# vstroebel/jpeg-encoder

Measured on NVIDIA B200. Metric: megapixels/sec encoded, byte-identical to the reference restatement, higher is better.
Workload: dtype u8 in / i32 arithmetic / i16 coefficients

## Files before the change

jpeg_encoder_b200/csrc/api.cu:

```cuda
#include <cuda.h>
#include <cuda_runtime.h>

#include <climits>
#include <cstdint>
#include <cstdio>
#include <cstdlib>
#include <algorithm>
#include <cstring>
#include <string>
#include <condition_variable>
#include <mutex>
#include <thread>
#include <utility>
#include <vector>

#include "../../include/jpegenc_b200.h"
#include "copy_pool.h"
#include "host.h"
#include "kernels.h"

using namespace jpgb;

namespace {

bool poison_alloc() {
    const char *e = std::getenv("JPGB_POISON_ALLOC");
    return e && e[0] == '1';
}

template <bool kPinned>
struct Buf {
    void *p = nullptr;
    size_t cap = 0;
    Buf() = default;
    Buf(Buf &&o) noexcept : p(std::exchange(o.p, nullptr)), cap(std::exchange(o.cap, 0)) {}
    Buf &operator=(Buf o) noexcept {
        std::swap(p, o.p);
        std::swap(cap, o.cap);
        return *this;
    }
    ~Buf() { if (p) kPinned ? cudaFreeHost(p) : cudaFree(p); }
    cudaError_t reserve(size_t bytes) {
        if (bytes <= cap) return cudaSuccess;
        *this = Buf();
        size_t want = bytes + bytes / 8 + 256;
        if (!kPinned) want = (want + 255) & ~(size_t)255;
        cudaError_t e = kPinned ? cudaMallocHost(&p, want) : cudaMalloc(&p, want);
        if (e != cudaSuccess) return p = nullptr, e;
        cap = want;
        if (poison_alloc()) {
            if (kPinned) std::memset(p, 0xFF, want);
            else if ((e = cudaMemset(p, 0xFF, want)) == cudaSuccess) e = cudaDeviceSynchronize();
        }
        return e;
    }
    template <typename T>
    T *as() const { return static_cast<T *>(p); }
};
using DevBuf = Buf<false>;
using PinnedBuf = Buf<true>;

struct PlanSig {
    jpgb_params p;
    jpgb_strip strip;
    uint32_t is_strip, planar;
};
inline PlanSig plan_sig(const Plan &plan) {
    PlanSig s;
    std::memset(&s, 0, sizeof(s));
    s.p.width = plan.p.width;
    s.p.height = plan.p.height;
    s.p.color_type = plan.p.color_type;
    s.p.quality = plan.p.quality;
    s.p.sampling = plan.p.sampling & 0x7F;
    for (int t = 0; t < 2; ++t) {
        s.p.qtable_kind[t] = plan.p.qtable_kind[t];
        if (plan.p.qtable_kind[t] == JPGB_QT_CUSTOM) std::memcpy(s.p.qtable_custom[t], plan.p.qtable_custom[t], sizeof(s.p.qtable_custom[t]));
    }
    s.p.progressive_scans = plan.p.progressive_scans;
    s.p.optimize_huffman = plan.p.optimize_huffman;
    s.p.restart_interval = plan.p.restart_interval;
    if (plan.is_strip) {
        s.strip.strip_index = plan.strip.strip_index;
        s.strip.n_strips = plan.strip.n_strips;
        s.strip.first_row = plan.strip.first_row;
        s.strip.rows = plan.strip.rows;
        s.strip.full_height = plan.strip.full_height;
    }
    s.is_strip = plan.is_strip;
    s.planar = plan.planar;
    return s;
}
struct CapKey {
    PlanSig sig;
    uint64_t raw_bytes;
    uint32_t n, pad;
};

struct Caps { uint64_t ustream, out, pool_units; };

struct GraphKey {
    PlanSig sig;
    uint64_t words[39];
};

struct GraphCache {
    struct Slot {
        cudaGraphExec_t exec = nullptr;
        GraphKey key{};
        uint32_t launches = 0;
        uint64_t used = 0;
    } slots[4];
    uint64_t clock = 0;
    bool ok = true;
    ~GraphCache() {
        for (Slot &s : slots)
            if (s.exec) cudaGraphExecDestroy(s.exec);
    }
    template <typename Enqueue>
    cudaError_t replay(const GraphKey &key, cudaStream_t st, uint32_t &launches, Enqueue &&enqueue, bool &replayed) {
        Slot *slot = nullptr, *victim = &slots[0];
        for (Slot &g : slots) {
            if (g.exec && std::memcmp(&g.key, &key, sizeof(key)) == 0) slot = &g;
            if (!g.exec || (victim->exec && g.used < victim->used)) victim = &g;
        }
        if (!slot) {
            if (victim->exec) cudaGraphExecDestroy(victim->exec), victim->exec = nullptr;
            const uint32_t launches_before = launches;
            cudaGraph_t graph = nullptr;
            const bool capturing = cudaStreamBeginCapture(st, cudaStreamCaptureModeThreadLocal) == cudaSuccess;
            const int rc = capturing ? enqueue() : JPGB_ERR_CUDA;
            if (capturing && cudaStreamEndCapture(st, &graph) == cudaSuccess && rc == JPGB_OK && graph &&
                cudaGraphInstantiate(&victim->exec, graph, 0) == cudaSuccess) {
                victim->key = key;
                victim->launches = launches - launches_before;
                slot = victim;
            } else {
                victim->exec = nullptr;
                ok = false;
            }
            if (graph) cudaGraphDestroy(graph);
            launches = launches_before;
            cudaGetLastError();
        }
        if (!slot) return cudaSuccess;
        slot->used = ++clock;
        const cudaError_t e = cudaGraphLaunch(slot->exec, st);
        if (e == cudaSuccess) launches += slot->launches, replayed = true;
        return e;
    }
};

}

struct jpgb_encoder {
    int device = 0;
    cudaStream_t stream = nullptr;
    bool own_stream = false;
    std::string err;
    DevBuf pixels, coef, huff, hdr, hdr_len, scratch, pool, chunk_bits, chunk_pool, chunk_bitpos, seglen, segpos, ustream, ffcount, ffpos,
        out, scan_tmp, hist, piece_off, out2, pixels2, status, hdr_parts;
    std::vector<uint8_t> last_tables;
    double ucap_ratio = 0;
    double pool_ratio = 0;
    PinnedBuf h_small, h_hist, h_tables, h_pieces, h_out, h_stage[2];
    cudaEvent_t ev_stage[2] = {};
    bool stage_busy[2] = {};
    CopyPool copy_pool;
    cudaStream_t s_h2d = nullptr, s_d2h = nullptr;
    std::vector<cudaEvent_t> ev_slice;
    cudaEvent_t ev_in[2] = {}, ev_out[2] = {}, ev_enc[2] = {};
    cudaEvent_t ev_wait = nullptr;
    bool timing = false;
    cudaEvent_t ev[JPGB_N_STAGES + 1][2] = {};
    bool ev_used[JPGB_N_STAGES] = {};
    float last_ms[JPGB_N_STAGES] = {};
    bool have_timing = false;
    uint32_t launches = 0;
    uint32_t last_piece_scans = 0;
    bool coef_tagged = false;
    PlanSig coef_sig{};
    const void *coef_pixels = nullptr;
    uint64_t coef_stride = 0;
    float coef_ms[2] = {0.f, 0.f};
    GraphCache graphs;
    bool have_caps = false;
    CapKey cap_key{};
    Caps caps{};
};

namespace {

int fail(jpgb_encoder *e, int code, const std::string &msg) {
    if (e) e->err = msg;
    return code;
}
int fail_cuda(jpgb_encoder *e, cudaError_t ce, const char *what) {
    return fail(e, JPGB_ERR_CUDA, std::string(what) + ": " + cudaGetErrorString(ce));
}
#define CK(call, what)                                        \
    do {                                                      \
        cudaError_t ce__ = (call);                            \
        if (ce__ != cudaSuccess) return fail_cuda(enc, ce__, what); \
    } while (0)

struct StageTimer {
    jpgb_encoder *enc;
    int stage;
    StageTimer(jpgb_encoder *e, int s) : enc(e), stage(s) {
        if (enc->timing) {
            if (!enc->ev_used[stage]) cudaEventRecord(enc->ev[stage][0], enc->stream);
        }
    }
    ~StageTimer() {
        if (enc->timing) {
            cudaEventRecord(enc->ev[stage][1], enc->stream);
            enc->ev_used[stage] = true;
        }
    }
};

void timing_begin(jpgb_encoder *enc) {
    for (int i = 0; i < JPGB_N_STAGES; ++i) enc->ev_used[i] = false;
    enc->have_timing = false;
    enc->launches = 0;
}
void timing_end(jpgb_encoder *enc) {
    if (!enc->timing) return;
    cudaStreamSynchronize(enc->stream);
    for (int i = 0; i < JPGB_N_STAGES; ++i) {
        enc->last_ms[i] = 0.f;
        if (enc->ev_used[i]) cudaEventElapsedTime(&enc->last_ms[i], enc->ev[i][0], enc->ev[i][1]);
    }
    enc->have_timing = true;
}

int validate_and_plan(jpgb_encoder *enc, const jpgb_params *p, size_t len_each, Plan &plan) {
    if (!p) return fail(enc, JPGB_ERR_BAD_PARAMS, "null params");
    if (p->color_type > JPGB_YCCK) return fail(enc, JPGB_ERR_BAD_PARAMS, "bad color_type");
    const size_t required = (size_t)p->width * p->height * (size_t)bytes_per_pixel(p->color_type);
    if (len_each < required) {
        char m[128];
        snprintf(m, sizeof(m), "Image data too small for dimensions and color_type: %zu need at least %zu", len_each, required);
        return fail(enc, JPGB_ERR_BAD_IMAGE_DATA, m);
    }
    const int rc = plan.build(*p);
    if (rc != JPGB_OK) return fail(enc, rc, rc == JPGB_ERR_ZERO_DIMENSIONS ? "Image dimensions must be non zero" : "invalid parameters");
    return JPGB_OK;
}

typedef CUresult (*MemGetAddressRangeFn)(CUdeviceptr *, size_t *, CUdeviceptr);
MemGetAddressRangeFn mem_get_address_range_fn() {
    static MemGetAddressRangeFn fn = [] {
        void *f = nullptr;
        cudaDriverEntryPointQueryResult q;
        if (cudaGetDriverEntryPoint("cuMemGetAddressRange", &f, cudaEnableDefault, &q) != cudaSuccess || q != cudaDriverEntryPointSuccess) f = nullptr;
        return reinterpret_cast<MemGetAddressRangeFn>(f);
    }();
    return fn;
}

int check_device_images(jpgb_encoder *enc, const Plan &plan, const jpgb_device_images &im, uint32_t n) {
    const uint64_t w = plan.p.width, h = plan.p.height;
    const bool planes = im.plane_stride != 0;
    const uint64_t row_bytes = planes ? w : w * (uint64_t)plan.bpp;
    char m[192];
    if (im.row_stride < row_bytes) {
        snprintf(m, sizeof(m), "row_stride %llu is shorter than a row (%llu bytes)", (unsigned long long)im.row_stride, (unsigned long long)row_bytes);
        return fail(enc, JPGB_ERR_BAD_PARAMS, m);
    }
    if (planes && im.plane_stride < w) {
        snprintf(m, sizeof(m), "plane_stride %llu is shorter than a row (%llu bytes)", (unsigned long long)im.plane_stride, (unsigned long long)w);
        return fail(enc, JPGB_ERR_BAD_PARAMS, m);
    }
    const uint8_t ct = plan.p.color_type;
    const uint64_t c_max = !planes ? 0 : (ct == JPGB_LUMA ? 0 : (plan.bpp == 3 || ct == JPGB_RGBA || ct == JPGB_BGRA) ? 2 : 3);
    uint64_t last = 0, t = 0;
    bool over = __builtin_mul_overflow((uint64_t)(n - 1), im.image_stride, &last);
    over |= __builtin_mul_overflow(c_max, im.plane_stride, &t) || __builtin_add_overflow(last, t, &last);
    over |= __builtin_mul_overflow(h - 1, im.row_stride, &t) || __builtin_add_overflow(last, t, &last);
    over |= __builtin_add_overflow(last, row_bytes - 1, &last);
    over |= __builtin_add_overflow((uint64_t)(uintptr_t)im.data, last, &t);
    if (over) return fail(enc, JPGB_ERR_BAD_PARAMS, "the described pixels extend beyond 64-bit addresses");
    CK(cudaSetDevice(enc->device), "cudaSetDevice");
    cudaPointerAttributes attr{};
    const bool known = cudaPointerGetAttributes(&attr, im.data) == cudaSuccess;
    cudaGetLastError();
    if (!known || !(attr.type == cudaMemoryTypeManaged || (attr.type == cudaMemoryTypeDevice && attr.device == enc->device)))
        return fail(enc, JPGB_ERR_BAD_PARAMS, "data is not device or managed memory of the context's device");
    MemGetAddressRangeFn range = mem_get_address_range_fn();
    CUdeviceptr base = 0;
    size_t size = 0;
    if (!range || range(&base, &size, (CUdeviceptr)(uintptr_t)im.data) != CUDA_SUCCESS)
        return fail(enc, JPGB_ERR_BAD_PARAMS, "no allocation is found at data");
    const uint64_t end = (uint64_t)(uintptr_t)im.data + last;
    if (end >= (uint64_t)base + size) {
        snprintf(m, sizeof(m), "the described pixels end %llu bytes past the end of the allocation that holds data",
                 (unsigned long long)(end + 1 - ((uint64_t)base + size)));
        return fail(enc, JPGB_ERR_BAD_PARAMS, m);
    }
    return JPGB_OK;
}

struct HeaderLayout {
    size_t hdr_stride = 0;
    uint32_t head_len = 0, tail_len = 0;
    int n_tables = 0;
};

int setup_header(jpgb_encoder *enc, const Plan &plan, uint32_t n, const uint32_t *given_hist, HeaderLayout &hl) {
    cudaStream_t st = enc->stream;
    const bool optimized = plan.p.optimize_huffman != 0;
    const uint32_t n_huff = optimized ? n : 1;
    const size_t tab_bytes = kHuffWordsPerImage * 4;
    CK(enc->huff.reserve((size_t)n_huff * tab_bytes), "alloc huffman tables");
    CK(enc->hdr_len.reserve((size_t)n_huff * 4), "alloc header lengths");
    std::vector<uint8_t> fresh;
    if (!optimized) {
        HuffTable tables[4];
        default_huffman_tables(reinterpret_cast<HuffTable(*)[2]>(tables));
        std::vector<uint8_t> h = plan.prefix;
        plan.frame_header(reinterpret_cast<const HuffTable(*)[2]>(tables), h);
        h.insert(h.end(), plan.scans[0].sos.begin(), plan.scans[0].sos.end());
        hl.hdr_stride = (h.size() + 15) & ~(size_t)15;
        fresh.assign(tab_bytes + hl.hdr_stride + 4, 0);
        CK(enc->h_tables.reserve(fresh.size()), "alloc tables (host)");
        for (int t = 0; t < 4; ++t)
            if (!tables[t].device_words(t & 1, reinterpret_cast<uint32_t *>(fresh.data() + (size_t)t * 1024)))
                return fail(enc, JPGB_ERR_HUFFMAN, "a Huffman code plus its value bits exceeds 31 bits");
        std::memcpy(fresh.data() + tab_bytes, h.data(), h.size());
        const uint32_t len = (uint32_t)h.size();
        std::memcpy(fresh.data() + tab_bytes + hl.hdr_stride, &len, 4);
    } else {
        std::vector<uint8_t> with;
        {
            HuffTable empty[2][2];
            const uint8_t none[16] = {0};
            for (auto &row : empty)
                for (HuffTable &e : row) e.set(none, nullptr, 0);
            with = plan.prefix;
            plan.frame_header(empty, with);
        }
        hl.n_tables = plan.ncomp >= 3 ? 2 : 1;
        size_t dht_at = plan.prefix.size();
        while (dht_at + 3 < with.size() && !(with[dht_at] == 0xFF && with[dht_at + 1] == 0xC4))
            dht_at += 2 + ((size_t)with[dht_at + 2] << 8 | with[dht_at + 3]);
        fresh.assign(with.begin(), with.begin() + dht_at);
        fresh.insert(fresh.end(), with.begin() + dht_at + (size_t)hl.n_tables * 2 * 21, with.end());
        fresh.insert(fresh.end(), plan.scans[0].sos.begin(), plan.scans[0].sos.end());
        hl.head_len = (uint32_t)dht_at;
        hl.tail_len = (uint32_t)(fresh.size() - dht_at);
        hl.hdr_stride = (fresh.size() + (size_t)hl.n_tables * 2 * (21 + 256) + 15) & ~(size_t)15;
        CK(enc->h_tables.reserve(fresh.size() + 16), "alloc header parts (host)");
        CK(enc->hdr_parts.reserve(fresh.size() + 16), "alloc header parts");
        fresh.push_back(0xA5);
        const size_t hist_words = (size_t)n * 2 * 2 * 257;
        CK(enc->hist.reserve(hist_words * 4), "alloc histogram");
        if (given_hist) {
            CK(enc->h_hist.reserve(hist_words * 4), "alloc histogram (host)");
            CK(cudaStreamSynchronize(st), "staging reuse sync");
            std::memcpy(enc->h_hist.p, given_hist, hist_words * 4);
            CK(cudaMemcpyAsync(enc->hist.p, enc->h_hist.p, hist_words * 4, cudaMemcpyHostToDevice, st), "upload histogram");
        }
    }
    CK(enc->hdr.reserve((size_t)n_huff * hl.hdr_stride), "alloc headers");
    if (enc->last_tables != fresh) {
        CK(cudaStreamSynchronize(st), "staging reuse sync");
        enc->last_tables = fresh;
        const uint8_t *hb = enc->h_tables.as<uint8_t>();
        std::memcpy(enc->h_tables.p, fresh.data(), fresh.size());
        if (!optimized) {
            CK(cudaMemcpyAsync(enc->huff.p, hb, tab_bytes, cudaMemcpyHostToDevice, st), "upload huffman tables");
            CK(cudaMemcpyAsync(enc->hdr.p, hb + tab_bytes, hl.hdr_stride, cudaMemcpyHostToDevice, st), "upload headers");
            CK(cudaMemcpyAsync(enc->hdr_len.p, hb + tab_bytes + hl.hdr_stride, 4, cudaMemcpyHostToDevice, st), "upload header lengths");
        } else {
            CK(cudaMemcpyAsync(enc->hdr_parts.p, hb, hl.head_len + hl.tail_len, cudaMemcpyHostToDevice, st), "upload header parts");
        }
    }
    return JPGB_OK;
}


Caps first_caps(const jpgb_encoder *enc, const CapKey &ck, uint64_t n_chunks) {
    const uint64_t raw_bytes = ck.raw_bytes;
    Caps c;
    c.ustream = (enc->ucap_ratio > 0 ? (uint64_t)(raw_bytes * enc->ucap_ratio) : raw_bytes / 3) + (uint64_t)ck.n * 4096 + 65536;
    c.out = c.ustream + c.ustream / 32 + 4096;
    c.pool_units = (enc->pool_ratio > 0 ? (uint64_t)(raw_bytes * enc->pool_ratio) : raw_bytes / 3) / 16 + n_chunks + 4096;
    if (enc->have_caps && std::memcmp(&enc->cap_key, &ck, sizeof(ck)) == 0) c = enc->caps;
    if (const char *tight = std::getenv("JPGB_TIGHT_CAPS")) {
        const std::string t = std::string(",") + tight + ",";
        if (t.find(",pool,") != std::string::npos) c.pool_units = 1;
        if (t.find(",stream,") != std::string::npos) c.ustream = kStuffChunk;
        if (t.find(",out,") != std::string::npos) c.out = 4096;
    }
    return c;
}

void grow_caps(Caps &c, const unsigned long long *status, uint64_t pool_used) {
    const uint64_t ubytes = status[kStatUnstuffed];
    if (status[kStatFlags] & kFlagPool) c.pool_units = pool_used + pool_used / 64 + 4096;
    if (status[kStatFlags] & kFlagStream) {
        c.ustream = ubytes + ubytes / 16 + 65536;
        c.out = c.ustream + c.ustream / 8 + 4096;
    } else if (status[kStatFlags] & kFlagOut) {
        c.out = ubytes + status[kStatDataFF] + 4096;
    }
}

void settle_caps(jpgb_encoder *enc, const CapKey &ck, const Caps &c, uint64_t ubytes, uint64_t total, uint64_t pool_used, uint64_t n_chunks) {
    auto settle = [](uint64_t cap, uint64_t need, uint64_t slack) {
        const uint64_t lo = need + need / 20 + slack / 2, hi = need + need * 2 / 5 + 2 * slack;
        return (cap >= lo && cap <= hi) ? cap : need + need * 3 / 20 + slack;
    };
    enc->cap_key = ck;
    enc->caps.ustream = settle(c.ustream, ubytes, (uint64_t)ck.n * 4096 + 65536);
    enc->caps.out = std::max(settle(c.out, total, 4096), enc->caps.ustream + enc->caps.ustream / 64);
    enc->caps.pool_units = settle(c.pool_units, pool_used, 4096);
    enc->have_caps = true;
    const double raw = (double)std::max<uint64_t>(ck.raw_bytes, 1);
    enc->pool_ratio = std::max(enc->pool_ratio * 0.98, 1.1 * (double)((pool_used > n_chunks ? pool_used - n_chunks : 0) * 16) / raw);
    enc->ucap_ratio = std::max(enc->ucap_ratio * 0.98, 1.15 * (double)ubytes / raw);
}

struct SequenceFlags { bool tables, given_hist, coder, poison, pieces; };

int enqueue_sequence(jpgb_encoder *enc, const Plan &plan, const DevPlan &hp, const EntropyBuffers &b, uint32_t n, const CoderLaunch &coder,
                     const HeaderLayout &hl, const SequenceFlags &f) {
    cudaStream_t st = enc->stream;
    const uint64_t n_chunks = (uint64_t)plan.chunks_per_image * n, n_segs = b.n_segs_total, n_pieces = b.ustream_cap / kStuffChunk;
    const StatusBlock sb = status_block(n, b.ustream_cap);
    unsigned long long *scan_err = b.status + kStatScanError;
    if (f.coder) {
        CK(cudaMemsetAsync(b.status, 0, 2 * kStatusWords * 8 + sb.mask_bytes, st), "clear status and raw mask");
    } else {
        CK(cudaMemsetAsync(b.status, 0, (kStatScanError + 1) * 8, st), "clear status");
        CK(cudaMemsetAsync(b.raw_mask, 0, sb.mask_bytes, st), "clear raw mask");
    }
    if (f.tables) {
        StageTimer t(enc, 1);
        if (!f.given_hist) {
            CK(cudaMemsetAsync(enc->hist.p, 0, (size_t)n * 2 * 2 * 257 * 4, st), "clear histogram");
            CK(launch_histogram(hp, b.coef, n, enc->hist.as<uint32_t>(), st), "histogram launch");
            enc->launches += 1;
        }
        CK(launch_build_tables(enc->hist.as<uint32_t>(), 1, hl.n_tables, n, enc->huff.as<uint32_t>(), enc->hdr_parts.as<uint8_t>(), hl.head_len,
                               enc->hdr_parts.as<uint8_t>() + hl.head_len, hl.tail_len, enc->hdr.as<uint8_t>(), (uint32_t)hl.hdr_stride,
                               enc->hdr_len.as<uint32_t>(), sb.table_status(b.file_off), st),
           "table build launch");
        enc->launches += 1;
    }
    if (f.coder) {
        StageTimer t(enc, 2);
        CK(launch_encode_chunks(b, hp, n, coder, st), "coding launch");
        enc->launches += 1;
        const bool few_chunks = n_chunks <= 4096, few_segs = n_segs <= 4096;
        if (!few_chunks) CK(launch_exclusive_scan(b.chunk_bits, b.chunk_bitpos, n_chunks, b.scan_tmp, st, &enc->launches, scan_err), "chunk position scan");
        if (few_segs) {
            CK(launch_positions(b, hp, n, few_chunks, st), "positions launch");
            enc->launches += 1;
        } else {
            if (few_chunks) CK(launch_exclusive_scan(b.chunk_bits, b.chunk_bitpos, n_chunks, b.scan_tmp, st, &enc->launches, scan_err), "chunk position scan");
            CK(launch_segment_lengths(b, hp, n, st), "segment length launch");
            CK(launch_exclusive_scan(b.seglen, b.segpos, n_segs, b.scan_tmp, st, &enc->launches, scan_err), "segment position scan");
            enc->launches += 1;
        }
    }
    {
        StageTimer t(enc, 3);
        if (f.poison) CK(cudaMemsetAsync(b.ustream, 0xFF, b.ustream_cap + 64, st), "poison stream");
        CK(launch_segment_leads(b, hp, n, st), "segment lead launch");
        CK(launch_place_chunks(b, hp, n, st), "placement launch");
        enc->launches += 2;
    }
    {
        StageTimer t(enc, 4);
        CK(launch_count_ff(b, st), "count ff launch");
        if (ff_scan_needed(b)) CK(launch_exclusive_scan(b.ffcount, b.ffpos, n_pieces, b.scan_tmp, st, &enc->launches, scan_err), "ff scan");
        CK(launch_stuff_scatter(b, hp, n, f.pieces ? enc->piece_off.as<unsigned long long>() : nullptr, st), "scatter launch");
        enc->launches += 2;
        if (f.pieces)
            CK(cudaMemcpyAsync(enc->h_pieces.p, enc->piece_off.p, (plan.scans.size() + 1) * 8, cudaMemcpyDeviceToHost, st), "read piece offsets");
        CK(cudaMemcpyAsync(enc->h_small.p, b.file_off, sb.readback_bytes(), cudaMemcpyDeviceToHost, st), "read file offsets and status");
    }
    return JPGB_OK;
}

GraphKey graph_key(const jpgb_encoder *enc, const PlanSig &sig, const EntropyBuffers &b, uint32_t n, const CoderLaunch &coder,
                   const HeaderLayout &hl, const SequenceFlags &f) {
    static_assert(sizeof(EntropyBuffers) == 26 * 8, "every field of EntropyBuffers takes part in the graph key");
    GraphKey k{{}, {
        (uint64_t)b.coef, (uint64_t)b.huff, (uint64_t)b.huff_per_image, (uint64_t)b.scratch, (uint64_t)b.pool, b.pool_cap,
        (uint64_t)b.chunk_bits, (uint64_t)b.chunk_pool, (uint64_t)b.chunk_bitpos, (uint64_t)b.seglen, (uint64_t)b.segpos,
        (uint64_t)b.hdr_len, (uint64_t)b.hdr, b.hdr_stride, (uint64_t)b.ustream, (uint64_t)b.raw_mask, (uint64_t)b.ffcount,
        (uint64_t)b.ffpos, (uint64_t)b.out, (uint64_t)b.file_off, (uint64_t)b.scan_tmp, b.ustream_cap, b.out_cap, b.n_segs_total,
        (uint64_t)b.status, b.scan_tmp_bytes,
        coder.grid, coder.smem, coder.scratch_bytes, n,
        (uint64_t)f.tables | (uint64_t)f.given_hist << 1 | (uint64_t)f.coder << 2 | (uint64_t)f.poison << 3 | (uint64_t)f.pieces << 4,
        hl.head_len, hl.tail_len, (uint64_t)hl.n_tables,
        (uint64_t)enc->hist.p, (uint64_t)enc->hdr_parts.p, (uint64_t)enc->piece_off.p, (uint64_t)enc->h_small.p, (uint64_t)enc->h_pieces.p}};
    std::memcpy(&k.sig, &sig, sizeof(sig));
    return k;
}

jpgb_device_images contiguous_images(const Plan &plan, const void *d_pixels, uint64_t image_stride) {
    const uint64_t row = (uint64_t)plan.p.width * (plan.planar ? 1 : plan.bpp);
    return {d_pixels, image_stride, row, plan.planar ? row * plan.p.height : 0};
}

void set_pixel_layout(StageAParams &ap, const Plan &plan, const jpgb_device_images &im) {
    ap.pixels = static_cast<const uint8_t *>(im.data);
    ap.image_stride = im.image_stride;
    ap.row_stride = im.row_stride;
    if (plan.planar) {
        ap.plane_stride = im.plane_stride;
    } else if (im.plane_stride && plan.ncomp > 1) {
        const uint8_t ct = plan.p.color_type;
        const bool bgr = ct == JPGB_BGR || ct == JPGB_BGRA;
        ap.channel_planar = 1;
        ap.plane_stride = im.plane_stride;
        for (int k = 0; k < 4; ++k) ap.plane_of[k] = (bgr && k < 3) ? 2 - k : k;
        if (ct == JPGB_BGR || ct == JPGB_RGBA || ct == JPGB_BGRA) {
            ap.color_type = JPGB_RGB;
            ap.bpp = 3;
        }
    }
}

int encode_device(jpgb_encoder *enc, const Plan &plan, const jpgb_device_images &images, uint32_t n, DevBuf &out,
                  std::vector<uint64_t> &offsets, std::vector<uint64_t> *piece_offsets = nullptr, const uint32_t *given_hist = nullptr,
                  bool coef_ready = false) {
    cudaStream_t st = enc->stream;
    DevPlan hp;
    plan.fill_device_plan(hp);

    const uint64_t n_segs = (uint64_t)plan.segs_per_image * n;
    const uint64_t n_chunks = (uint64_t)plan.chunks_per_image * n;

    CK(enc->coef.reserve(plan.blocks_per_image * n * 128), "alloc coefficients");
    if (!coef_ready) {
        enc->coef_tagged = false;
        StageAParams ap;
        plan.fill_stage_a(ap);
        set_pixel_layout(ap, plan, images);
        ap.coef = enc->coef.as<int16_t>();
        StageTimer t(enc, 0);
        CK(launch_stage_a(ap, n, st), "stage A launch");
        enc->launches += 1;
    }

    HeaderLayout hl;
    int rc = setup_header(enc, plan, n, given_hist, hl);
    if (rc != JPGB_OK) return rc;

    CK(enc->chunk_bits.reserve(n_chunks * 4), "alloc chunk sizes");
    CK(enc->chunk_pool.reserve(n_chunks * 4), "alloc chunk places");
    CK(enc->chunk_bitpos.reserve((n_chunks + 1) * 8), "alloc chunk positions");
    CK(enc->seglen.reserve(n_segs * 4), "alloc seglen");
    CK(enc->segpos.reserve((n_segs + 1) * 8), "alloc segpos");
    CoderLaunch coder{};
    CK(coder_launch_config(hp, n, coder), "coder configuration");
    CK(enc->scratch.reserve(coder.scratch_bytes), "alloc coder scratch");
    CK(enc->h_small.reserve(status_block(n, 0).readback_bytes()), "alloc readback");
    if (piece_offsets) {
        CK(enc->piece_off.reserve((plan.scans.size() + 1) * 8), "alloc piece offsets");
        CK(enc->h_pieces.reserve((plan.scans.size() + 1) * 8), "alloc piece offsets (host)");
    }

    EntropyBuffers b{};
    b.coef = enc->coef.as<int16_t>();
    b.huff = enc->huff.as<uint32_t>();
    b.huff_per_image = plan.p.optimize_huffman != 0 ? 1 : 0;
    b.scratch = enc->scratch.as<uint32_t>();
    b.chunk_bits = enc->chunk_bits.as<uint32_t>();
    b.chunk_pool = enc->chunk_pool.as<uint32_t>();
    b.chunk_bitpos = enc->chunk_bitpos.as<unsigned long long>();
    b.seglen = enc->seglen.as<uint32_t>();
    b.segpos = enc->segpos.as<unsigned long long>();
    b.hdr_len = enc->hdr_len.as<uint32_t>();
    b.hdr = enc->hdr.as<uint8_t>();
    b.hdr_stride = (uint32_t)hl.hdr_stride;
    b.n_segs_total = n_segs;

    CapKey ck;
    std::memset(&ck, 0, sizeof(ck));
    ck.sig = plan_sig(plan);
    ck.raw_bytes = (uint64_t)plan.p.width * plan.p.height * plan.bpp * n;
    ck.n = n;
    Caps caps = first_caps(enc, ck, n_chunks);
    const char *poison_env = std::getenv("JPGB_POISON_STREAM");
    uint64_t ubytes = 0, total = 0, pool_used = 0;
    bool coded = false;
    for (int attempt = 0;; ++attempt) {
        caps.ustream = (caps.ustream + kStuffChunk - 1) / kStuffChunk * kStuffChunk;
        const uint64_t n_pieces = caps.ustream / kStuffChunk;
        const StatusBlock sb = status_block(n, caps.ustream);
        CK(enc->ustream.reserve(caps.ustream + 64), "alloc unstuffed stream");
        CK(enc->status.reserve(sb.bytes()), "alloc status and raw mask");
        CK(enc->ffcount.reserve((n_pieces + 1) * 4), "alloc ff counts");
        CK(enc->ffpos.reserve((n_pieces + 2) * 8), "alloc ff positions");
        CK(enc->scan_tmp.reserve(scan_tmp_bytes(std::max<uint64_t>(n_pieces, std::max(n_chunks, n_segs)))), "alloc scan scratch");
        CK(enc->pool.reserve(caps.pool_units * 16), "alloc chunk pool");
        CK(out.reserve(caps.out + 64), "alloc output");
        b.pool = enc->pool.as<uint32_t>();
        b.pool_cap = caps.pool_units;
        b.ustream = enc->ustream.as<uint8_t>();
        b.file_off = sb.file_off(enc->status.p);
        b.status = sb.status(enc->status.p);
        b.raw_mask = sb.raw_mask(enc->status.p);
        b.ffcount = enc->ffcount.as<uint32_t>();
        b.ffpos = enc->ffpos.as<unsigned long long>();
        b.scan_tmp = enc->scan_tmp.p;
        b.out = out.as<uint8_t>();
        b.ustream_cap = caps.ustream;
        b.out_cap = caps.out;
        const SequenceFlags f{plan.p.optimize_huffman != 0 && attempt == 0, given_hist != nullptr, !coded, poison_env && poison_env[0] == '1',
                              piece_offsets != nullptr};
        auto enqueue = [&] { return enqueue_sequence(enc, plan, hp, b, n, coder, hl, f); };
        bool replayed = false;
        if (attempt == 0 && enc->graphs.ok && !enc->timing)
            CK(enc->graphs.replay(graph_key(enc, ck.sig, b, n, coder, hl, f), st, enc->launches, enqueue, replayed), "graph launch");
        if (!replayed) {
            rc = enqueue();
            if (rc != JPGB_OK) return rc;
        }
        CK(cudaStreamSynchronize(st), "final sync");
        const unsigned long long *status = sb.status(enc->h_small.p);
        if (status[kStatScanError]) return fail(enc, JPGB_ERR_CUDA, "internal: prefix-sum look-back timed out");
        if (status[kStatFlags] & kFlagSegment4G) return fail(enc, JPGB_ERR_BAD_PARAMS, "a scan segment exceeds 4 GiB (use a restart interval)");
        if (f.tables && (sb.table_status(enc->h_small.p)[kStatFlags] & kFlagHuffmanLong))
            return fail(enc, JPGB_ERR_HUFFMAN, "an optimized Huffman code does not fit (longer than 32 bits, or code plus value bits beyond 31)");
        ubytes = status[kStatUnstuffed];
        if (f.coder) pool_used = status[kStatPoolCursor];
        if (status[kStatFlags] == 0) {
            total = ubytes + status[kStatDataFF];
            break;
        }
        if (attempt >= 3) return fail(enc, JPGB_ERR_CUDA, "internal: buffer capacity retry did not converge");
        coded = !(status[kStatFlags] & kFlagPool);
        grow_caps(caps, status, pool_used);
    }
    settle_caps(enc, ck, caps, ubytes, total, pool_used, n_chunks);
    if (piece_offsets) {
        piece_offsets->assign(enc->h_pieces.as<uint64_t>(), enc->h_pieces.as<uint64_t>() + plan.scans.size() + 1);
        enc->last_piece_scans = (uint32_t)plan.scans.size();
    }
    offsets.assign(enc->h_small.as<uint64_t>(), enc->h_small.as<uint64_t>() + n + 1);
    if (offsets[n] != total) return fail(enc, JPGB_ERR_CUDA, "internal: file offsets disagree with stream size");
    return JPGB_OK;
}

constexpr size_t kStageBytes = 16u << 20;
cudaError_t upload_host(jpgb_encoder *enc, void *d_dst, const uint8_t *src, size_t bytes, cudaStream_t s) {
    cudaPointerAttributes attr{};
    const bool pinned = cudaPointerGetAttributes(&attr, src) == cudaSuccess && (attr.type == cudaMemoryTypeHost || attr.type == cudaMemoryTypeManaged);
    cudaGetLastError();
    if (pinned || bytes <= 65536) return cudaMemcpyAsync(d_dst, src, bytes, cudaMemcpyHostToDevice, s);
    size_t piece = kStageBytes;
    if (bytes >= kStageBytes && bytes < 2 * kStageBytes) piece = ((bytes / 2 + (1u << 20) - 1) >> 20) << 20;
    unsigned hw = std::thread::hardware_concurrency();
    if (const char *e = std::getenv("JPGB_COPY_THREADS")) hw = (unsigned)std::max(1, std::atoi(e));
    for (size_t off = 0, k = 0; off < bytes; off += piece, ++k) {
        const int b = (int)(k & 1);
        const size_t n = std::min(piece, bytes - off);
        cudaError_t e = enc->h_stage[b].reserve(kStageBytes);
        if (e != cudaSuccess) return e;
        if (enc->stage_busy[b]) {
            e = cudaEventSynchronize(enc->ev_stage[b]);
            if (e != cudaSuccess) return e;
        }
        unsigned threads = (unsigned)std::min<size_t>(4, n >> 22);
        if (hw && threads > hw) threads = hw;
        enc->copy_pool.copy(enc->h_stage[b].p, src + off, n, threads);
        e = cudaMemcpyAsync(static_cast<uint8_t *>(d_dst) + off, enc->h_stage[b].p, n, cudaMemcpyHostToDevice, s);
        if (e != cudaSuccess) return e;
        e = cudaEventRecord(enc->ev_stage[b], s);
        if (e != cudaSuccess) return e;
        enc->stage_busy[b] = true;
    }
    return cudaSuccess;
}

int encode_host_pipelined(jpgb_encoder *enc, const Plan &plan, const uint8_t *const *pixels, uint32_t n,
                          std::vector<uint64_t> &offsets) {
    const size_t img_bytes = (size_t)plan.p.width * plan.p.height * plan.bpp;
    const size_t stride = (img_bytes + 255) & ~(size_t)255;
    uint32_t chunk = (uint32_t)std::max<size_t>(1, (96u << 20) / stride);
    chunk = std::min(chunk, n);
    const uint32_t n_chunks = (n + chunk - 1) / chunk;
    CK(enc->pixels.reserve(stride * chunk), "alloc pixels");
    if (n_chunks > 1) CK(enc->pixels2.reserve(stride * chunk), "alloc pixels");
    CK(enc->h_out.reserve(std::max<size_t>(img_bytes * n / 3, 1 << 20)), "alloc pinned output");
    offsets.assign(1, 0);
    cudaStream_t st = enc->stream;

    if (n == 1 && !plan.planar && img_bytes >= (48u << 20)) {
        const size_t row_bytes = (size_t)plan.p.width * plan.bpp;
        const uint32_t mcu_px = 8 * plan.vmax;
        uint32_t rows_per_slice = (uint32_t)std::max<size_t>(1, (32u << 20) / (row_bytes * mcu_px));
        rows_per_slice = (rows_per_slice + 3) & ~3u;
        const uint32_t n_slices = (plan.mcu_rows + rows_per_slice - 1) / rows_per_slice;
        CK(enc->pixels.reserve(stride), "alloc pixels");
        CK(enc->coef.reserve(plan.blocks_per_image * 128), "alloc coefficients");
        enc->coef_tagged = false;
        while (enc->ev_slice.size() < n_slices) {
            cudaEvent_t e;
            CK(cudaEventCreateWithFlags(&e, cudaEventDisableTiming), "create event");
            enc->ev_slice.push_back(e);
        }
        StageAParams ap;
        plan.fill_stage_a(ap);
        for (uint32_t k = 0; k < n_slices; ++k) {
            const size_t r0 = (size_t)k * rows_per_slice * mcu_px, r1 = std::min<size_t>(plan.p.height, r0 + (size_t)rows_per_slice * mcu_px);
            CK(upload_host(enc, enc->pixels.as<uint8_t>() + r0 * row_bytes, pixels[0] + r0 * row_bytes, (r1 - r0) * row_bytes, enc->s_h2d), "upload slice");
            CK(cudaEventRecord(enc->ev_slice[k], enc->s_h2d), "record slice");
        }
        for (uint32_t k = 0; k < n_slices; ++k) {
            const size_t r0 = (size_t)k * rows_per_slice * mcu_px, r1 = std::min<size_t>(plan.p.height, r0 + (size_t)rows_per_slice * mcu_px);
            StageAParams sp = ap;
            sp.pixels = enc->pixels.as<uint8_t>() + r0 * row_bytes;
            sp.coef = enc->coef.as<int16_t>();
            sp.image_stride = stride;
            sp.height = (int)(r1 - r0);
            sp.mcu_row0 = (int)(k * rows_per_slice);
            sp.mcu_rows = (int)std::min<uint32_t>(rows_per_slice, plan.mcu_rows - k * rows_per_slice);
            CK(cudaStreamWaitEvent(st, enc->ev_slice[k], 0), "wait slice");
            CK(launch_stage_a(sp, 1, st), "stage A launch");
            enc->launches += 1;
        }
        std::vector<uint64_t> off;
        const int rc = encode_device(enc, plan, contiguous_images(plan, enc->pixels.p, stride), 1, enc->out, off, nullptr, nullptr, true);
        if (rc != JPGB_OK) return rc;
        CK(enc->h_out.reserve(std::max<size_t>(off[1], 1 << 20)), "alloc pinned output");
        CK(cudaMemcpyAsync(enc->h_out.p, enc->out.p, off[1], cudaMemcpyDeviceToHost, st), "download file");
        CK(cudaStreamSynchronize(st), "download sync");
        offsets.push_back(off[1]);
        return JPGB_OK;
    }

    auto upload = [&](uint32_t c) -> cudaError_t {
        DevBuf &px = (c & 1) ? enc->pixels2 : enc->pixels;
        const uint32_t lo = c * chunk, hi = std::min(n, lo + chunk);
        if (c >= 2) {
            cudaError_t e = cudaStreamWaitEvent(enc->s_h2d, enc->ev_enc[c & 1], 0);
            if (e != cudaSuccess) return e;
        }
        for (uint32_t i = lo; i < hi; ++i) {
            cudaError_t e = upload_host(enc, px.as<uint8_t>() + stride * (i - lo), pixels[i], img_bytes, enc->s_h2d);
            if (e != cudaSuccess) return e;
        }
        return cudaEventRecord(enc->ev_in[c & 1], enc->s_h2d);
    };

    {
        StageTimer t(enc, 5);
        CK(upload(0), "upload pixels");
    }
    uint64_t total = 0;
    for (uint32_t c = 0; c < n_chunks; ++c) {
        const uint32_t lo = c * chunk, hi = std::min(n, lo + chunk), cn = hi - lo;
        if (c + 1 < n_chunks) CK(upload(c + 1), "upload pixels");
        DevBuf &px = (c & 1) ? enc->pixels2 : enc->pixels;
        DevBuf &ob = (c & 1) ? enc->out2 : enc->out;
        CK(cudaStreamWaitEvent(st, enc->ev_in[c & 1], 0), "wait upload");
        if (c >= 2) CK(cudaStreamWaitEvent(st, enc->ev_out[c & 1], 0), "wait download");
        std::vector<uint64_t> off;
        const int rc = encode_device(enc, plan, contiguous_images(plan, px.p, stride), cn, ob, off);
        if (rc != JPGB_OK) return rc;
        CK(cudaEventRecord(enc->ev_enc[c & 1], st), "record encode");
        const uint64_t bytes = off[cn];
        if (total + bytes > enc->h_out.cap) {
            CK(cudaStreamSynchronize(enc->s_d2h), "download sync");
            PinnedBuf bigger;
            CK(bigger.reserve((total + bytes) * 2), "grow pinned output");
            std::memcpy(bigger.p, enc->h_out.p, total);
            std::swap(enc->h_out, bigger);
        }
        CK(cudaMemcpyAsync(enc->h_out.as<uint8_t>() + total, ob.p, bytes, cudaMemcpyDeviceToHost, enc->s_d2h), "download files");
        CK(cudaEventRecord(enc->ev_out[c & 1], enc->s_d2h), "record download");
        for (uint32_t i = 0; i < cn; ++i) offsets.push_back(total + off[i + 1]);
        total += bytes;
    }
    {
        StageTimer t(enc, 6);
        CK(cudaStreamSynchronize(enc->s_d2h), "download sync");
    }
    return JPGB_OK;
}

int encode_host_batch(jpgb_encoder *enc, const jpgb_params *p, const uint8_t *const *pixels, size_t len_each, uint32_t n,
                      uint8_t **outs, size_t *out_lens, const uint8_t **pinned_base, uint64_t *pinned_offsets) {
    if (!enc) return JPGB_ERR_BAD_PARAMS;
    const bool pinned_api = pinned_base != nullptr;
    if (!pixels || n == 0 || (pinned_api ? !pinned_offsets : (!outs || !out_lens))) return fail(enc, JPGB_ERR_BAD_PARAMS, "null argument");
    if (!pinned_api)
        for (uint32_t i = 0; i < n; ++i) outs[i] = nullptr, out_lens[i] = 0;
    Plan plan;
    int rc = validate_and_plan(enc, p, len_each, plan);
    if (rc != JPGB_OK) return rc;
    CK(cudaSetDevice(enc->device), "cudaSetDevice");
    const bool was_timing = enc->timing;
    enc->timing = false;
    timing_begin(enc);
    std::vector<uint64_t> off;
    rc = encode_host_pipelined(enc, plan, pixels, n, off);
    enc->timing = was_timing;
    if (rc != JPGB_OK) return rc;
    if (pinned_api) {
        *pinned_base = enc->h_out.as<uint8_t>();
        std::memcpy(pinned_offsets, off.data(), (size_t)(n + 1) * 8);
        return JPGB_OK;
    }
    for (uint32_t i = 0; i < n; ++i) {
        const size_t sz = (size_t)(off[i + 1] - off[i]);
        outs[i] = static_cast<uint8_t *>(std::malloc(sz ? sz : 1));
        if (!outs[i]) {
            for (uint32_t k = 0; k < i; ++k) std::free(outs[k]), outs[k] = nullptr;
            return fail(enc, JPGB_ERR_NOMEM, "out of host memory");
        }
        out_lens[i] = sz;
        std::memcpy(outs[i], enc->h_out.as<uint8_t>() + off[i], sz);
    }
    return JPGB_OK;
}

}

extern "C" {

void jpgb_params_default(jpgb_params *p, uint8_t quality) {
    std::memset(p, 0, sizeof(*p));
    p->quality = quality;
    p->sampling = quality < 90 ? 0x22 : 0x11;
    p->density_unit = 0;
    p->density_x = p->density_y = 1;
}

int jpgb_encoder_create(int device, void *cuda_stream, jpgb_encoder **out) {
    if (!out) return JPGB_ERR_BAD_PARAMS;
    *out = nullptr;
    int count = 0;
    if (cudaGetDeviceCount(&count) != cudaSuccess || device < 0 || device >= count) return JPGB_ERR_CUDA;
    cudaDeviceProp prop;
    if (cudaGetDeviceProperties(&prop, device) != cudaSuccess) return JPGB_ERR_CUDA;
    if (prop.major != 10) return JPGB_ERR_CUDA;
    if (cudaSetDevice(device) != cudaSuccess) return JPGB_ERR_CUDA;
    jpgb_encoder *e = new (std::nothrow) jpgb_encoder();
    if (!e) return JPGB_ERR_NOMEM;
    e->device = device;
    if (cuda_stream) {
        e->stream = static_cast<cudaStream_t>(cuda_stream);
    } else {
        if (cudaStreamCreateWithFlags(&e->stream, cudaStreamNonBlocking) != cudaSuccess) {
            delete e;
            return JPGB_ERR_CUDA;
        }
        e->own_stream = true;
    }
    for (int i = 0; i < JPGB_N_STAGES; ++i)
        for (int k = 0; k < 2; ++k) cudaEventCreate(&e->ev[i][k]);
    cudaStreamCreateWithFlags(&e->s_h2d, cudaStreamNonBlocking);
    cudaStreamCreateWithFlags(&e->s_d2h, cudaStreamNonBlocking);
    for (int i = 0; i < 2; ++i) {
        cudaEventCreateWithFlags(&e->ev_in[i], cudaEventDisableTiming);
        cudaEventCreateWithFlags(&e->ev_out[i], cudaEventDisableTiming);
        cudaEventCreateWithFlags(&e->ev_enc[i], cudaEventDisableTiming);
        cudaEventCreateWithFlags(&e->ev_stage[i], cudaEventDisableTiming);
    }
    cudaEventCreateWithFlags(&e->ev_wait, cudaEventDisableTiming);
    *out = e;
    return JPGB_OK;
}

void jpgb_encoder_destroy(jpgb_encoder *e) {
    if (!e) return;
    cudaSetDevice(e->device);
    cudaStreamSynchronize(e->stream);
    if (e->s_h2d) cudaStreamDestroy(e->s_h2d);
    if (e->s_d2h) cudaStreamDestroy(e->s_d2h);
    for (cudaEvent_t ev : e->ev_slice) cudaEventDestroy(ev);
    for (int i = 0; i < 2; ++i) {
        if (e->ev_in[i]) cudaEventDestroy(e->ev_in[i]);
        if (e->ev_out[i]) cudaEventDestroy(e->ev_out[i]);
        if (e->ev_enc[i]) cudaEventDestroy(e->ev_enc[i]);
        if (e->ev_stage[i]) cudaEventDestroy(e->ev_stage[i]);
    }
    if (e->ev_wait) cudaEventDestroy(e->ev_wait);
    for (int i = 0; i < JPGB_N_STAGES; ++i)
        for (int k = 0; k < 2; ++k)
            if (e->ev[i][k]) cudaEventDestroy(e->ev[i][k]);
    if (e->own_stream) cudaStreamDestroy(e->stream);
    delete e;
}

const char *jpgb_last_error(const jpgb_encoder *e) { return e ? e->err.c_str() : "no encoder"; }

int jpgb_encode(jpgb_encoder *enc, const jpgb_params *p, const uint8_t *pixels, size_t len, uint8_t **out, size_t *out_len) {
    if (!out || !out_len) return JPGB_ERR_BAD_PARAMS;
    *out = nullptr;
    *out_len = 0;
    const uint8_t *px[1] = {pixels};
    return encode_host_batch(enc, p, px, len, 1, out, out_len, nullptr, nullptr);
}

void jpgb_free(void *buf) { std::free(buf); }

static int encode_planar_pinned(jpgb_encoder *enc, const jpgb_params *p, const uint8_t *const planes[4], size_t plane_len, size_t *out_len) {
    if (!p || !planes) return fail(enc, JPGB_ERR_BAD_PARAMS, "null argument");
    const uint8_t ct = p->color_type;
    if (ct != JPGB_LUMA && ct != JPGB_YCBCR && ct != JPGB_CMYK && ct != JPGB_YCCK)
        return fail(enc, JPGB_ERR_BAD_PARAMS, "planar input takes a JPEG colour type: Luma, Ycbcr, Cmyk or Ycck");
    const size_t plane_bytes = (size_t)p->width * p->height;
    if (plane_len < plane_bytes) return fail(enc, JPGB_ERR_BAD_IMAGE_DATA, "plane shorter than width*height");
    Plan plan;
    plan.planar = true;
    const int rc = plan.build(*p);
    if (rc != JPGB_OK) return fail(enc, rc, rc == JPGB_ERR_ZERO_DIMENSIONS ? "Image dimensions must be non zero" : "invalid parameters");
    CK(cudaSetDevice(enc->device), "cudaSetDevice");
    timing_begin(enc);
    const size_t stride = (plane_bytes * plan.ncomp + 255) & ~(size_t)255;
    CK(enc->pixels.reserve(stride), "alloc planes");
    for (int c = 0; c < plan.ncomp; ++c) {
        if (!planes[c]) return fail(enc, JPGB_ERR_BAD_PARAMS, "null plane");
        CK(upload_host(enc, enc->pixels.as<uint8_t>() + plane_bytes * c, planes[c], plane_bytes, enc->stream), "upload plane");
    }
    std::vector<uint64_t> off;
    const int rc2 = encode_device(enc, plan, contiguous_images(plan, enc->pixels.p, stride), 1, enc->out, off);
    if (rc2 != JPGB_OK) return rc2;
    const size_t sz = (size_t)off[1];
    CK(enc->h_out.reserve(sz ? sz : 1), "alloc pinned output");
    CK(cudaMemcpyAsync(enc->h_out.p, enc->out.p, sz, cudaMemcpyDeviceToHost, enc->stream), "download file");
    CK(cudaStreamSynchronize(enc->stream), "download sync");
    *out_len = sz;
    timing_end(enc);
    return JPGB_OK;
}

int jpgb_encode_planar(jpgb_encoder *enc, const jpgb_params *p, const uint8_t *const planes[4], size_t plane_len, uint8_t **out,
                       size_t *out_len) {
    if (!enc) return JPGB_ERR_BAD_PARAMS;
    if (!out || !out_len) return fail(enc, JPGB_ERR_BAD_PARAMS, "null argument");
    *out = nullptr;
    *out_len = 0;
    size_t sz = 0;
    const int rc = encode_planar_pinned(enc, p, planes, plane_len, &sz);
    if (rc != JPGB_OK) return rc;
    *out = static_cast<uint8_t *>(std::malloc(sz ? sz : 1));
    if (!*out) return fail(enc, JPGB_ERR_NOMEM, "out of host memory");
    std::memcpy(*out, enc->h_out.p, sz);
    *out_len = sz;
    return JPGB_OK;
}

int jpgb_encode_planar_to_sink(jpgb_encoder *enc, const jpgb_params *p, const uint8_t *const planes[4], size_t plane_len,
                               jpgb_write_all_fn write_all, void *user) {
    if (!enc) return JPGB_ERR_BAD_PARAMS;
    if (!write_all) return fail(enc, JPGB_ERR_BAD_PARAMS, "null sink");
    size_t sz = 0;
    const int rc = encode_planar_pinned(enc, p, planes, plane_len, &sz);
    if (rc != JPGB_OK) return rc;
    if (write_all(user, enc->h_out.as<uint8_t>(), sz) != 0) return fail(enc, JPGB_ERR_SINK, "sink write_all failed");
    return JPGB_OK;
}

int jpgb_encode_to_sink(jpgb_encoder *enc, const jpgb_params *p, const uint8_t *pixels, size_t len, jpgb_write_all_fn write_all,
                        void *user) {
    if (!enc) return JPGB_ERR_BAD_PARAMS;
    if (!write_all) return fail(enc, JPGB_ERR_BAD_PARAMS, "null sink");
    const uint8_t *px[1] = {pixels};
    const uint8_t *files = nullptr;
    uint64_t offs[2] = {0, 0};
    const int rc = encode_host_batch(enc, p, px, len, 1, nullptr, nullptr, &files, offs);
    if (rc != JPGB_OK) return rc;
    if (write_all(user, files + offs[0], (size_t)(offs[1] - offs[0])) != 0) return fail(enc, JPGB_ERR_SINK, "sink write_all failed");
    return JPGB_OK;
}

int jpgb_encode_batch(jpgb_encoder *enc, const jpgb_params *p, const uint8_t *const *pixels, size_t len_each, uint32_t n,
                      uint8_t **outs, size_t *out_lens) {
    return encode_host_batch(enc, p, pixels, len_each, n, outs, out_lens, nullptr, nullptr);
}

int jpgb_encode_batch_pinned(jpgb_encoder *enc, const jpgb_params *p, const uint8_t *const *pixels, size_t len_each, uint32_t n,
                             const uint8_t **files, uint64_t *offsets) {
    if (!files) return JPGB_ERR_BAD_PARAMS;
    return encode_host_batch(enc, p, pixels, len_each, n, nullptr, nullptr, files, offsets);
}

int jpgb_encode_batch_device(jpgb_encoder *enc, const jpgb_params *p, const void *d_pixels, size_t image_stride, uint32_t n,
                             const void **d_files, uint64_t *offsets) {
    if (!enc) return JPGB_ERR_BAD_PARAMS;
    if (!d_pixels || !d_files || !offsets || n == 0) return fail(enc, JPGB_ERR_BAD_PARAMS, "null argument");
    Plan plan;
    int rc = validate_and_plan(enc, p, image_stride, plan);
    if (rc != JPGB_OK) return rc;
    CK(cudaSetDevice(enc->device), "cudaSetDevice");
    timing_begin(enc);
    std::vector<uint64_t> off;
    rc = encode_device(enc, plan, contiguous_images(plan, d_pixels, image_stride), n, enc->out, off);
    if (rc != JPGB_OK) return rc;
    timing_end(enc);
    std::memcpy(offsets, off.data(), (size_t)(n + 1) * 8);
    *d_files = enc->out.p;
    return JPGB_OK;
}

int jpgb_encode_batch_device_strided(jpgb_encoder *enc, const jpgb_params *p, const jpgb_device_images *images, uint32_t n,
                                     const void **d_files, uint64_t *offsets) {
    if (!enc) return JPGB_ERR_BAD_PARAMS;
    enc->launches = 0;
    if (!images || !images->data || !d_files || !offsets || n == 0) return fail(enc, JPGB_ERR_BAD_PARAMS, "null argument");
    Plan plan;
    int rc = validate_and_plan(enc, p, SIZE_MAX, plan);
    if (rc != JPGB_OK) return rc;
    rc = check_device_images(enc, plan, *images, n);
    if (rc != JPGB_OK) return rc;
    plan.planar = images->plane_stride != 0 && (p->color_type == JPGB_YCBCR || p->color_type == JPGB_YCCK);
    timing_begin(enc);
    std::vector<uint64_t> off;
    rc = encode_device(enc, plan, *images, n, enc->out, off);
    if (rc != JPGB_OK) return rc;
    timing_end(enc);
    std::memcpy(offsets, off.data(), (size_t)(n + 1) * 8);
    *d_files = enc->out.p;
    return JPGB_OK;
}

int jpgb_encoder_wait_stream(jpgb_encoder *enc, void *stream) {
    if (!enc) return JPGB_ERR_BAD_PARAMS;
    cudaStream_t s = static_cast<cudaStream_t>(stream);
    if (s == enc->stream) return JPGB_OK;
    CK(cudaSetDevice(enc->device), "cudaSetDevice");
    CK(cudaEventRecord(enc->ev_wait, s), "record the caller's stream");
    CK(cudaStreamWaitEvent(enc->stream, enc->ev_wait, 0), "wait for the caller's stream");
    return JPGB_OK;
}

int jpgb_scan_count(const jpgb_params *p, uint32_t *n_scans) {
    if (!p || !n_scans) return JPGB_ERR_BAD_PARAMS;
    Plan plan;
    const int rc = plan.build(*p);
    if (rc != JPGB_OK) return rc;
    *n_scans = (uint32_t)plan.scans.size();
    return JPGB_OK;
}

int jpgb_plan_strips(const jpgb_params *p, uint32_t max_strips, jpgb_strip *strips, uint32_t *n_strips) {
    if (!p || !strips || !n_strips || max_strips == 0) return JPGB_ERR_BAD_PARAMS;
    Plan plan;
    const int rc = plan.build(*p);
    if (rc != JPGB_OK) return rc;
    const uint32_t R = p->restart_interval;
    if (R == 0) return JPGB_ERR_BAD_PARAMS;
    auto gcd = [](uint64_t a, uint64_t b) { while (b) { const uint64_t t = a % b; a = b; b = t; } return a; };
    uint64_t step = 1;
    for (const Scan &s : plan.scans) {
        const uint64_t upr = s.comp < 0 ? plan.mcu_cols : (uint64_t)plan.comps[s.comp].v * plan.true_w[s.comp];
        const uint64_t need = R / gcd(R, upr);
        step = step / gcd(step, need) * need;
    }
    const uint64_t groups = (plan.mcu_rows + step - 1) / step;
    uint32_t n = (uint32_t)std::min<uint64_t>(max_strips, groups);
    if (n == 0) n = 1;
    const uint32_t rows_per_mcu = 8 * plan.vmax;
    uint64_t g0 = 0;
    for (uint32_t i = 0; i < n; ++i) {
        const uint64_t g1 = groups * (i + 1) / n;
        const uint64_t r0 = g0 * step * rows_per_mcu, r1 = std::min<uint64_t>(g1 * step * rows_per_mcu, p->height);
        strips[i].strip_index = i;
        strips[i].n_strips = n;
        strips[i].first_row = (uint16_t)r0;
        strips[i].rows = (uint16_t)(r1 - r0);
        strips[i].full_height = p->height;
        g0 = g1;
    }
    *n_strips = n;
    return JPGB_OK;
}

static int encode_strip(jpgb_encoder *enc, const jpgb_params *p, const jpgb_strip *strip, const void *d_pixels, const uint32_t *hist_total,
                        const void **d_bytes, uint64_t *piece_offsets) {
    if (!enc) return JPGB_ERR_BAD_PARAMS;
    if (!p || !strip || !d_pixels || !d_bytes || !piece_offsets) return fail(enc, JPGB_ERR_BAD_PARAMS, "null argument");
    if (p->color_type > JPGB_YCCK) return fail(enc, JPGB_ERR_BAD_PARAMS, "bad color_type");
    if ((p->optimize_huffman != 0) != (hist_total != nullptr))
        return fail(enc, JPGB_ERR_BAD_PARAMS, "optimized tables with strips take the whole image's histogram (jpgb_encode_strip_device_optimized); other settings take none");
    Plan plan;
    const int rc = plan.build(*p, strip);
    if (rc != JPGB_OK) return fail(enc, rc, "settings or strip geometry do not allow strip encoding (needs restart intervals aligned in every scan)");
    CK(cudaSetDevice(enc->device), "cudaSetDevice");
    timing_begin(enc);
    std::vector<uint64_t> off, pieces;
    const size_t stride = (size_t)p->width * strip->rows * bytes_per_pixel(p->color_type);
    bool reuse = false;
    if (hist_total && enc->coef_tagged && enc->coef_pixels == d_pixels && enc->coef_stride == uint64_t(stride)) {
        const PlanSig sig = plan_sig(plan);
        reuse = std::memcmp(&sig, &enc->coef_sig, sizeof(sig)) == 0;
    }
    const int rc2 = encode_device(enc, plan, contiguous_images(plan, d_pixels, stride), 1, enc->out, off, &pieces, hist_total, reuse);
    enc->coef_tagged = false;
    if (rc2 != JPGB_OK) return rc2;
    timing_end(enc);
    if (reuse && enc->timing) {
        enc->last_ms[0] += enc->coef_ms[0];
        enc->last_ms[1] += enc->coef_ms[1];
    }
    std::memcpy(piece_offsets, pieces.data(), pieces.size() * 8);
    *d_bytes = enc->out.p;
    return JPGB_OK;
}

int jpgb_encode_strip_device(jpgb_encoder *enc, const jpgb_params *p, const jpgb_strip *strip, const void *d_pixels,
                             const void **d_bytes, uint64_t *piece_offsets) {
    return encode_strip(enc, p, strip, d_pixels, nullptr, d_bytes, piece_offsets);
}

int jpgb_encode_strip_device_optimized(jpgb_encoder *enc, const jpgb_params *p, const jpgb_strip *strip, const void *d_pixels,
                                       const uint32_t hist_total[JPGB_HIST_WORDS], const void **d_bytes, uint64_t *piece_offsets) {
    if (enc && !hist_total) return fail(enc, JPGB_ERR_BAD_PARAMS, "null histogram");
    return encode_strip(enc, p, strip, d_pixels, hist_total, d_bytes, piece_offsets);
}

int jpgb_strip_histogram_device(jpgb_encoder *enc, const jpgb_params *p, const jpgb_strip *strip, const void *d_pixels,
                                uint32_t hist[JPGB_HIST_WORDS], int16_t edge_dc[8]) {
    if (!enc) return JPGB_ERR_BAD_PARAMS;
    if (!p || !strip || !d_pixels || !hist || !edge_dc) return fail(enc, JPGB_ERR_BAD_PARAMS, "null argument");
    if (p->color_type > JPGB_YCCK || !p->optimize_huffman) return fail(enc, JPGB_ERR_BAD_PARAMS, "strip histograms belong to optimized Huffman tables");
    Plan plan;
    const int rc = plan.build(*p, strip);
    if (rc != JPGB_OK) return fail(enc, rc, "settings or strip geometry do not allow strip encoding (needs restart intervals aligned in every scan)");
    CK(cudaSetDevice(enc->device), "cudaSetDevice");
    cudaStream_t st = enc->stream;
    DevPlan hp;
    plan.fill_device_plan(hp);
    StageAParams ap;
    plan.fill_stage_a(ap);
    CK(enc->coef.reserve(plan.blocks_per_image * 128), "alloc coefficients");
    ap.pixels = static_cast<const uint8_t *>(d_pixels);
    ap.coef = enc->coef.as<int16_t>();
    ap.image_stride = (size_t)p->width * strip->rows * bytes_per_pixel(p->color_type);
    timing_begin(enc);
    {
        StageTimer t(enc, 0);
        CK(launch_stage_a(ap, 1, st), "stage A launch");
    }
    const size_t hist_bytes = JPGB_HIST_WORDS * 4;
    CK(enc->hist.reserve(hist_bytes), "alloc histogram");
    CK(enc->h_hist.reserve(hist_bytes + 16), "alloc histogram (host)");
    {
        StageTimer t(enc, 1);
        CK(cudaMemsetAsync(enc->hist.p, 0, hist_bytes, st), "clear histogram");
        CK(launch_histogram(hp, enc->coef.as<int16_t>(), 1, enc->hist.as<uint32_t>(), st), "histogram launch");
    }
    enc->launches = 2;
    CK(cudaMemcpyAsync(enc->h_hist.p, enc->hist.p, hist_bytes, cudaMemcpyDeviceToHost, st), "download histogram");
    int16_t *edge = reinterpret_cast<int16_t *>(enc->h_hist.as<uint8_t>() + hist_bytes);
    std::memset(edge, 0, 16);
    for (int c = 0; c < plan.ncomp; ++c) {
        const uint64_t first = plan.block_off[c], last = plan.block_off[c] + (uint64_t)plan.true_w[c] * plan.true_h[c] - 1;
        CK(cudaMemcpyAsync(edge + c, enc->coef.as<int16_t>() + first * 64, 2, cudaMemcpyDeviceToHost, st), "read edge DC");
        CK(cudaMemcpyAsync(edge + 4 + c, enc->coef.as<int16_t>() + last * 64, 2, cudaMemcpyDeviceToHost, st), "read edge DC");
    }
    CK(cudaStreamSynchronize(st), "histogram sync");
    std::memcpy(hist, enc->h_hist.p, hist_bytes);
    std::memcpy(edge_dc, edge, 16);
    enc->coef_sig = plan_sig(plan);
    enc->coef_pixels = d_pixels;
    enc->coef_stride = uint64_t(ap.image_stride);
    enc->coef_tagged = true;
    timing_end(enc);
    enc->coef_ms[0] = enc->timing ? enc->last_ms[0] : 0.f;
    enc->coef_ms[1] = enc->timing ? enc->last_ms[1] : 0.f;
    return JPGB_OK;
}

int jpgb_merge_strip_histograms(const jpgb_params *p, uint32_t n_strips, const uint32_t hist_sum[JPGB_HIST_WORDS], const int16_t *edge_dc,
                                uint32_t hist_total[JPGB_HIST_WORDS]) {
    if (!p || !hist_sum || !edge_dc || !hist_total || n_strips == 0) return JPGB_ERR_BAD_PARAMS;
    Plan plan;
    const int rc = plan.build(*p);
    if (rc != JPGB_OK) return rc;
    std::memcpy(hist_total, hist_sum, JPGB_HIST_WORDS * 4);
    auto category = [](int diff) {
        int a = (int16_t)diff;
        a = a < 0 ? -a : a;
        int n = 0;
        while (a) ++n, a >>= 1;
        return n;
    };
    for (uint32_t s = 1; s < n_strips; ++s)
        for (int c = 0; c < plan.ncomp; ++c) {
            uint32_t *dc = hist_total + (size_t)plan.comps[c].dc_table * 2 * 257;
            const int first = edge_dc[s * 8 + c], prev_last = edge_dc[(s - 1) * 8 + 4 + c];
            dc[category(first)] -= 1;
            dc[category(first - prev_last)] += 1;
        }
    return JPGB_OK;
}

int jpgb_gather_target_create(jpgb_encoder *enc, size_t capacity, void **d_target, uint8_t ipc_handle[64]) {
    if (!enc) return JPGB_ERR_BAD_PARAMS;
    if (!d_target || !ipc_handle || capacity == 0) return fail(enc, JPGB_ERR_BAD_PARAMS, "null argument");
    static_assert(sizeof(cudaIpcMemHandle_t) == 64, "the C ABI carries the IPC handle as 64 bytes");
    CK(cudaSetDevice(enc->device), "cudaSetDevice");
    void *p = nullptr;
    CK(cudaMalloc(&p, capacity + 64), "alloc gather target");
    cudaIpcMemHandle_t h;
    const cudaError_t ce = cudaIpcGetMemHandle(&h, p);
    if (ce != cudaSuccess) {
        cudaFree(p);
        return fail_cuda(enc, ce, "cudaIpcGetMemHandle");
    }
    std::memcpy(ipc_handle, &h, 64);
    *d_target = p;
    return JPGB_OK;
}

int jpgb_gather_target_open(jpgb_encoder *enc, const uint8_t ipc_handle[64], void **d_target) {
    if (!enc) return JPGB_ERR_BAD_PARAMS;
    if (!d_target || !ipc_handle) return fail(enc, JPGB_ERR_BAD_PARAMS, "null argument");
    CK(cudaSetDevice(enc->device), "cudaSetDevice");
    cudaIpcMemHandle_t h;
    std::memcpy(&h, ipc_handle, 64);
    void *p = nullptr;
    CK(cudaIpcOpenMemHandle(&p, h, cudaIpcMemLazyEnablePeerAccess), "cudaIpcOpenMemHandle (peer access over NVLink)");
    *d_target = p;
    return JPGB_OK;
}

int jpgb_gather_target_close(jpgb_encoder *enc, void *d_target, int opened_from_handle) {
    if (!enc) return JPGB_ERR_BAD_PARAMS;
    if (!d_target) return JPGB_OK;
    CK(cudaSetDevice(enc->device), "cudaSetDevice");
    CK(cudaStreamSynchronize(enc->stream), "sync before releasing the gather target");
    if (opened_from_handle) CK(cudaIpcCloseMemHandle(d_target), "cudaIpcCloseMemHandle");
    else CK(cudaFree(d_target), "free gather target");
    return JPGB_OK;
}

int jpgb_last_piece_offsets_device(jpgb_encoder *enc, const uint64_t **d_offsets, uint32_t *n_scans) {
    if (!enc) return JPGB_ERR_BAD_PARAMS;
    if (!d_offsets || !n_scans || !enc->piece_off.p || enc->last_piece_scans == 0) return fail(enc, JPGB_ERR_BAD_PARAMS, "no strip has been encoded on this context");
    *d_offsets = enc->piece_off.as<uint64_t>();
    *n_scans = enc->last_piece_scans;
    return JPGB_OK;
}

int jpgb_gather_place_pieces(jpgb_encoder *enc, void *d_target, size_t target_capacity, const uint64_t *d_table, uint32_t world, uint32_t rank,
                             uint64_t *d_total) {
    if (!enc) return JPGB_ERR_BAD_PARAMS;
    if (!d_target || !d_table || world == 0 || rank >= world || enc->last_piece_scans == 0) return fail(enc, JPGB_ERR_BAD_PARAMS, "bad gather arguments");
    CK(cudaSetDevice(enc->device), "cudaSetDevice");
    CK(launch_place_pieces(enc->out.as<uint8_t>(), static_cast<uint8_t *>(d_target), target_capacity, reinterpret_cast<const unsigned long long *>(d_table),
                           world, rank, enc->last_piece_scans, reinterpret_cast<unsigned long long *>(d_total), enc->stream),
       "piece placement launch");
    return JPGB_OK;
}

int jpgb_download(jpgb_encoder *enc, const void *d_src, size_t n, void *host_dst) {
    if (!enc) return JPGB_ERR_BAD_PARAMS;
    if (n == 0) return JPGB_OK;
    if (!d_src || !host_dst) return fail(enc, JPGB_ERR_BAD_PARAMS, "null argument");
    CK(cudaSetDevice(enc->device), "cudaSetDevice");
    CK(cudaMemcpyAsync(host_dst, d_src, n, cudaMemcpyDeviceToHost, enc->stream), "download");
    CK(cudaStreamSynchronize(enc->stream), "download sync");
    return JPGB_OK;
}

int jpgb_coef_layout_for(const jpgb_params *p, jpgb_coef_layout *l) {
    if (!p || !l) return JPGB_ERR_BAD_PARAMS;
    Plan plan;
    const int rc = plan.build(*p);
    if (rc != JPGB_OK) return rc;
    std::memset(l, 0, sizeof(*l));
    l->n_components = (uint32_t)plan.ncomp;
    for (int c = 0; c < plan.ncomp; ++c) {
        l->blocks_w[c] = plan.pad_w[c];
        l->blocks_h[c] = plan.pad_h[c];
        l->true_w[c] = plan.true_w[c];
        l->true_h[c] = plan.true_h[c];
        l->block_offset[c] = plan.block_off[c];
        l->slot_base[c] = plan.slot_base[c];
        l->comp_h[c] = plan.comps[c].h;
        l->comp_v[c] = plan.comps[c].v;
    }
    l->blocks_per_image = plan.blocks_per_image;
    l->mcu_order = plan.mode == Mode::Interleaved;
    l->mcu_cols = plan.mcu_cols;
    l->mcu_rows = plan.mcu_rows;
    l->blocks_per_mcu = plan.bpu_interleaved;
    return JPGB_OK;
}

int jpgb_stage_a_device(jpgb_encoder *enc, const jpgb_params *p, const void *d_pixels, size_t image_stride, uint32_t n, void *d_coef) {
    if (!enc) return JPGB_ERR_BAD_PARAMS;
    if (!d_pixels || !d_coef || n == 0) return fail(enc, JPGB_ERR_BAD_PARAMS, "null argument");
    Plan plan;
    const int rc = validate_and_plan(enc, p, image_stride, plan);
    if (rc != JPGB_OK) return rc;
    CK(cudaSetDevice(enc->device), "cudaSetDevice");
    StageAParams ap;
    plan.fill_stage_a(ap);
    ap.pixels = static_cast<const uint8_t *>(d_pixels);
    ap.coef = static_cast<int16_t *>(d_coef);
    ap.image_stride = image_stride;
    enc->launches = 0;
    CK(launch_stage_a(ap, n, enc->stream), "stage A launch");
    enc->launches = 1;
    return JPGB_OK;
}

void jpgb_encoder_set_timing(jpgb_encoder *enc, int enabled) {
    if (enc) enc->timing = enabled != 0;
}
int jpgb_encoder_last_timing(const jpgb_encoder *enc, float ms[JPGB_N_STAGES]) {
    if (!enc || !enc->have_timing) return JPGB_ERR_BAD_PARAMS;
    std::memcpy(ms, enc->last_ms, sizeof(enc->last_ms));
    return JPGB_OK;
}
uint32_t jpgb_encoder_last_launch_count(const jpgb_encoder *enc) { return enc ? enc->launches : 0; }

int jpgb_build_header(const jpgb_params *p, uint8_t *buf, size_t cap, size_t *len) {
    if (!p || !len) return JPGB_ERR_BAD_PARAMS;
    Plan plan;
    const int rc = plan.build(*p);
    if (rc != JPGB_OK) return rc;
    HuffTable huff[2][2];
    default_huffman_tables(huff);
    std::vector<uint8_t> h = plan.prefix;
    plan.frame_header(huff, h);
    h.insert(h.end(), plan.scans[0].sos.begin(), plan.scans[0].sos.end());
    *len = h.size();
    if (buf) std::memcpy(buf, h.data(), std::min(cap, h.size()));
    return JPGB_OK;
}

int jpgb_optimized_huffman_table(const uint32_t freq[257], uint8_t length[16], uint8_t values[256], uint32_t *n_values) {
    if (!freq || !length || !values || !n_values) return JPGB_ERR_BAD_PARAMS;
    HuffTable t;
    if (!t.set_optimized(freq)) return JPGB_ERR_HUFFMAN;
    std::memcpy(length, t.length, 16);
    std::memcpy(values, t.values.data(), t.values.size());
    *n_values = (uint32_t)t.values.size();
    return JPGB_OK;
}

int jpgb_optimized_huffman_tables_device(jpgb_encoder *enc, const uint32_t *freq, uint32_t n, int ac, uint8_t *lengths, uint8_t *values,
                                         uint32_t *n_values, uint32_t *words, int *status) {
    if (!enc) return JPGB_ERR_BAD_PARAMS;
    if (!freq || !lengths || !values || !n_values || !words || !status || n == 0) return fail(enc, JPGB_ERR_BAD_PARAMS, "null argument");
    CK(cudaSetDevice(enc->device), "cudaSetDevice");
    cudaStream_t st = enc->stream;
    DevBuf d_hist, d_words, d_dht, d_len, d_bad;
    std::vector<uint8_t> dht((size_t)n * 277);
    std::vector<uint32_t> len(n), bad(n);
    cudaError_t e = d_hist.reserve((size_t)n * 257 * 4);
    if (e == cudaSuccess) e = d_words.reserve((size_t)n * 1024);
    if (e == cudaSuccess) e = d_dht.reserve((size_t)n * 277);
    if (e == cudaSuccess) e = d_len.reserve((size_t)n * 4);
    if (e == cudaSuccess) e = d_bad.reserve((size_t)n * 4);
    if (e == cudaSuccess) e = cudaMemcpyAsync(d_hist.p, freq, (size_t)n * 257 * 4, cudaMemcpyHostToDevice, st);
    if (e == cudaSuccess) e = launch_build_single_tables(d_hist.as<uint32_t>(), n, ac, d_words.as<uint32_t>(), d_dht.as<uint8_t>(), d_len.as<uint32_t>(), d_bad.as<uint32_t>(), st);
    if (e == cudaSuccess) e = cudaMemcpyAsync(words, d_words.p, (size_t)n * 1024, cudaMemcpyDeviceToHost, st);
    if (e == cudaSuccess) e = cudaMemcpyAsync(dht.data(), d_dht.p, dht.size(), cudaMemcpyDeviceToHost, st);
    if (e == cudaSuccess) e = cudaMemcpyAsync(len.data(), d_len.p, (size_t)n * 4, cudaMemcpyDeviceToHost, st);
    if (e == cudaSuccess) e = cudaMemcpyAsync(bad.data(), d_bad.p, (size_t)n * 4, cudaMemcpyDeviceToHost, st);
    if (e == cudaSuccess) e = cudaStreamSynchronize(st);
    if (e != cudaSuccess) return fail_cuda(enc, e, "device table build");
    for (uint32_t i = 0; i < n; ++i) {
        status[i] = bad[i] ? JPGB_ERR_HUFFMAN : JPGB_OK;
        n_values[i] = bad[i] ? 0 : len[i] - 21;
        std::memcpy(lengths + (size_t)i * 16, dht.data() + (size_t)i * 277 + 5, 16);
        std::memcpy(values + (size_t)i * 256, dht.data() + (size_t)i * 277 + 21, 256);
    }
    return JPGB_OK;
}

const char *jpgb_version(void) { return "jpeg-encoder_b200 0.1 (sm_100a; parity target: jpeg-encoder 0.7.0)"; }

}
```

jpeg_encoder_b200/csrc/entropy.cu:

```cuda

#include "kernels.h"

namespace jpgb {
namespace {

__device__ __forceinline__ int find_scan_by_seg(const DevPlan &P, unsigned s) {
    int lo = 0, hi = P.n_scans - 1;
    while (lo < hi) {
        const int mid = (lo + hi + 1) >> 1;
        if (P.scans[mid].seg_base <= s) lo = mid;
        else hi = mid - 1;
    }
    return lo;
}
__device__ __forceinline__ int find_scan_by_chunk(const DevPlan &P, unsigned c) {
    int lo = 0, hi = P.n_scans - 1;
    while (lo < hi) {
        const int mid = (lo + hi + 1) >> 1;
        if (P.scans[mid].chunk_base <= c) lo = mid;
        else hi = mid - 1;
    }
    return lo;
}

__device__ __forceinline__ void value_code(int v, int &size, uint32_t &bits) {
    const int a = v < 0 ? -v : v;
    int top;
    asm("bfind.u32 %0, %1;" : "=r"(top) : "r"(a));
    size = top + 1;
    uint32_t mask;
    asm("bmsk.clamp.b32 %0, 0, %1;" : "=r"(mask) : "r"(size));
    bits = (uint32_t)(v + (v >> 31)) & mask;
}

__device__ __forceinline__ unsigned nonzero16x2(unsigned x) {
    unsigned r;
    asm("min.u16x2 %0, %1, %2;" : "=r"(r) : "r"(x), "r"(0x00010001u));
    return r;
}

template <int T>
struct BitSink {
    unsigned long long acc = 0;
    int n = 0;
    unsigned off = 0;
    uint32_t *slot0;

    __device__ __forceinline__ BitSink(uint32_t *scratch, int visit) : slot0(scratch + visit) {}
    __device__ __forceinline__ void put(uint32_t code, int len) {
        acc = (acc << len) | code;
        n += len;
        if (n >= 32) {
            n -= 32;
            *reinterpret_cast<uint32_t *>(reinterpret_cast<char *>(slot0) + off) = (uint32_t)(acc >> n);
            off += T * 4;
        }
    }
    __device__ __forceinline__ unsigned finish() {
        if (n > 0) *reinterpret_cast<uint32_t *>(reinterpret_cast<char *>(slot0) + off) = (uint32_t)(acc << (32 - n));
        return off / (T * 4) * 32 + n;
    }
};

constexpr uint32_t kCodeBits = 0x07FFFFFFu;

constexpr int kStageStride = 72;
constexpr int kAsmWordsProg = 3072;

__device__ __forceinline__ unsigned long long zrl_markers(unsigned long long m, int first_ac) {
    const unsigned long long z = m | (1ull << (first_ac - 1));
    unsigned long long s = z;
    s |= s << 1;
    s |= s << 2;
    s |= s << 4;
    const unsigned long long s16 = s | (s << 8);
    const unsigned long long s32 = s16 | (s16 << 16);
    const unsigned long long s48 = s32 | (s16 << 32);
    unsigned long long marks = ((z << 16) & ~s16) | ((z << 32) & ~s32) | ((z << 48) & ~s48);
    const int top = 63 - __clzll((long long)m);
    marks &= top > 0 ? (~0ull >> (64 - top)) : 0ull;
    return marks;
}

template <int BASE, int T>
__device__ __forceinline__ void code_half(unsigned m, int &next, unsigned c_shared, const uint32_t *__restrict__ tab, BitSink<T> &sink) {
#pragma unroll 1
    while (m) {
        int p;
        asm("bfind.u32 %0, %1;" : "=r"(p) : "r"(m));
        unsigned bit;
        asm("bmsk.clamp.b32 %0, %1, 1;" : "=r"(bit) : "r"(p));
        m ^= bit;
        const int k = BASE + 31 - p;
        int v;
        asm("ld.shared.s16 %0, [%1];" : "=r"(v) : "r"(c_shared + 2 * k));
        const int run = k - next;
        next = k + 1;
        int size;
        uint32_t bits;
        value_code(v, size, bits);
        const uint32_t e = (tab + run * 16)[size];
        sink.put((e & kCodeBits) | bits, (int)(e >> 27));
    }
}
template <int T>
__device__ __forceinline__ void code_nonzeros(unsigned lo_rev, unsigned hi_rev, int first_ac, int se, const int16_t *__restrict__ c,
                                              const uint32_t *__restrict__ tab, BitSink<T> &sink) {
    int next = first_ac;
    const unsigned c_shared = (unsigned)__cvta_generic_to_shared(c);
    code_half<0, T>(lo_rev, next, c_shared, tab, sink);
    code_half<32, T>(hi_rev, next, c_shared, tab, sink);
    if (next <= se) {
        const uint32_t e = tab[0];
        sink.put(e & kCodeBits, (int)(e >> 27));
    }
}

struct __align__(16) ItemInfo {
    unsigned long long img, blk0, chunk_index0;
    unsigned v_in_seg0, n_valid, group;
    int done;
};

template <int T, bool FULL>
struct CoderSmem {
    static constexpr int kCoefBytes = T * kStageStride * 2;
    static constexpr int kAsmWords = FULL ? kCoefBytes / 4 : kAsmWordsProg;
    static constexpr int oAsm = FULL ? 0 : kCoefBytes;
    static constexpr int oAc = kCoefBytes + (FULL ? 0 : kAsmWordsProg * 4);
    static constexpr int oDc = oAc + 2048;
    static constexpr int oSlot = oDc + 256;
    static constexpr int oBin = oSlot + 128;
    static constexpr int oNb = oBin + 256;
    static constexpr int oOrder = oNb + T * 4;
    static constexpr int oWsum = oOrder + T * 2;
    static constexpr int oItem = oWsum + 64;
    static constexpr int kBytes = oItem + 2 * 64;
};

__host__ __device__ constexpr int coder_min_ctas(int T, bool full) { return full && T >= 128 ? 1280 / T : 1024 / T; }

template <int T, bool FULL>
__global__ void __launch_bounds__(T, coder_min_ctas(T, FULL)) encode_chunks_kernel(const __grid_constant__ EntropyBuffers b, const __grid_constant__ DevPlan P,
                                                          unsigned long long n_items) {
    using L = CoderSmem<T, FULL>;
    extern __shared__ __align__(16) unsigned char smem[];
    int16_t *coef = reinterpret_cast<int16_t *>(smem);
    uint32_t *asmbuf = reinterpret_cast<uint32_t *>(smem + L::oAsm);
    uint32_t *ac_tab = reinterpret_cast<uint32_t *>(smem + L::oAc);
    uint2 *dc_tab = reinterpret_cast<uint2 *>(smem + L::oDc);
    uint32_t *slot_tab = reinterpret_cast<uint32_t *>(smem + L::oSlot);
    uint32_t *bin = reinterpret_cast<uint32_t *>(smem + L::oBin);
    uint32_t *nbv = reinterpret_cast<uint32_t *>(smem + L::oNb);
    auto visit_meta = [&](int v) { return reinterpret_cast<uint4 *>(smem + v * (kStageStride * 2) + 128); };
    uint16_t *order = reinterpret_cast<uint16_t *>(smem + L::oOrder);
    uint32_t *wsum = reinterpret_cast<uint32_t *>(smem + L::oWsum);
    ItemInfo *items = reinterpret_cast<ItemInfo *>(smem + L::oItem);

    const int tid = threadIdx.x, lane = tid & 31, warp = tid >> 5;
    uint32_t *scratch = b.scratch + (size_t)blockIdx.x * (T * kSlotWords);
    long long tab_img = -1;
    for (int i = tid; i < 64; i += T) bin[i] = 0;
    if (tid < kMaxSlots) slot_tab[tid] = (unsigned)P.comp_tbl[P.slot_comp[tid]] | (unsigned)P.slot_back[tid] << 8 | (unsigned)P.slot_first[tid] << 16;
    auto decode = [&](unsigned long long ticket, ItemInfo &it) {
        it.done = ticket >= n_items;
        if (it.done) return;
        unsigned long long img;
        unsigned r;
        if ((ticket >> 32) == 0) {
            unsigned q;
            divmod((unsigned)ticket, P.div_items, q, r);
            img = q;
        } else {
            img = ticket / P.items_per_image;
            r = (unsigned)(ticket - img * P.items_per_image);
        }
        int g = 0;
        while (g + 1 < P.n_groups && r >= P.groups[g + 1].item_base) ++g;
        const DevGroup &G = P.groups[g];
        unsigned seg, chunk;
        divmod(r - G.item_base, G.div_cps, seg, chunk);
        const unsigned long long seg_start = (unsigned long long)seg * G.seg_visits;
        const unsigned long long v0 = seg_start + (unsigned long long)chunk * T;
        unsigned long long seg_end = seg_start + G.seg_visits;
        if (seg_end > G.n_visits) seg_end = G.n_visits;
        it.img = img;
        it.group = (unsigned)g;
        it.v_in_seg0 = chunk * T;
        it.n_valid = v0 < seg_end ? (unsigned)(seg_end - v0 < (unsigned long long)T ? seg_end - v0 : T) : 0u;
        it.blk0 = img * P.blocks_per_image + G.block_base + v0;
        it.chunk_index0 = img * P.chunks_per_image + (r - G.item_base);
    };
    unsigned long long next_ticket = 0;
    if (tid == 0) {
        decode(atomicAdd(b.status + kStatTicket, 1ull), items[0]);
        next_ticket = atomicAdd(b.status + kStatTicket, 1ull);
    }

    for (unsigned round = 0;; ++round) {
        __syncthreads();
        const ItemInfo it = items[round & 1];
        if (it.done) break;
        if (tid == 0) {
            decode(next_ticket, items[(round & 1) ^ 1]);
            next_ticket = atomicAdd(b.status + kStatTicket, 1ull);
        }
        if (it.n_valid == 0) {
            for (int j = tid; j < P.spg; j += T) {
                const unsigned long long ci = it.chunk_index0 + P.scans[it.group + j * P.n_groups].chunk_base;
                b.chunk_bits[ci] = 0;
                b.chunk_pool[ci] = 0;
            }
            continue;
        }
        const DevGroup &G = P.groups[it.group];
        const bool valid = (unsigned)tid < it.n_valid;

        const long long want_tab = b.huff_per_image ? (long long)it.img : 0;
        if (want_tab != tab_img) {
            const uint32_t *set = b.huff + (size_t)want_tab * kHuffWordsPerImage;
            for (int i = tid; i < 512; i += T) {
                ac_tab[i] = __ldg(set + (i >> 8) * 512 + 256 + (i & 255));
            }
            if (tid < 32) {
                const uint32_t e = __ldg(set + (tid >> 4) * 512 + (tid & 15));
                dc_tab[tid] = make_uint2(e & kCodeBits, e >> 27);
            }
            tab_img = want_tab;
        }

        const int16_t *src_blocks = b.coef + it.blk0 * 64;
        {
            const unsigned pieces = it.n_valid * 8;
            const char *g = reinterpret_cast<const char *>(src_blocks) + (size_t)tid * 16;
            const unsigned d = (unsigned)__cvta_generic_to_shared(coef) + (tid >> 3) * (kStageStride * 2) + (tid & 7) * 16;
            if (it.n_valid == T) {
#pragma unroll
                for (int k = 0; k < 8; ++k)
                    asm volatile("cp.async.cg.shared.global [%0], [%1], 16;" ::"r"(d + k * (T / 8) * (kStageStride * 2)), "l"(g + k * T * 16) : "memory");
            } else {
#pragma unroll
                for (int k = 0; k < 8; ++k)
                    if ((unsigned)(tid + k * T) < pieces)
                        asm volatile("cp.async.cg.shared.global [%0], [%1], 16;" ::"r"(d + k * (T / 8) * (kStageStride * 2)), "l"(g + k * T * 16) : "memory");
            }
            asm volatile("cp.async.wait_all;" ::: "memory");
        }
        __syncthreads();

        unsigned long long m_all = 0;
        int dcdiff = 0, tbl = 0;
        if (valid) {
            const uint4 *mine = reinterpret_cast<const uint4 *>(coef + tid * kStageStride);
            unsigned m_lo = 0, m_hi = 0;
#pragma unroll
            for (int w = 0; w < 8; ++w) {
                const uint4 q = mine[w];
                unsigned byte = __dp2a_lo(nonzero16x2(q.x), 0x0201u, 0u);
                byte = __dp2a_lo(nonzero16x2(q.y), 0x0804u, byte);
                byte = __dp2a_lo(nonzero16x2(q.z), 0x2010u, byte);
                byte = __dp2a_lo(nonzero16x2(q.w), 0x8040u, byte);
                if (w < 4) m_lo |= byte << (8 * w);
                else m_hi |= byte << (8 * (w - 4));
            }
            m_all = (((unsigned long long)m_hi << 32) | m_lo) & ~1ull;
            const unsigned v_in_seg = it.v_in_seg0 + tid;
            unsigned unit = v_in_seg, slot = 0;
            if (G.bpu > 1) divmod(v_in_seg, G.div_bpu, unit, slot);
            const unsigned sinfo = G.comp < 0 ? slot_tab[slot] : ((unsigned)P.comp_tbl[G.comp] | 0x10100u);
            tbl = sinfo & 0xFF;
            const int back = (sinfo >> 8) & 0xFF;
            const bool first_of_comp = (sinfo >> 16) != 0;
            int prev = 0;
            if (!(unit == 0 && first_of_comp)) prev = tid >= back ? (int)coef[(tid - back) * kStageStride] : (int)__ldg(src_blocks + ((long long)tid - back) * 64);
            dcdiff = (int)(int16_t)(coef[tid * kStageStride] - prev);
        }

        for (int j = 0; j < (FULL ? 1 : P.spg); ++j) {
            const DevScan &S = P.scans[it.group + j * P.n_groups];
            const int ss = FULL ? 0 : S.ss, se = FULL ? 63 : S.se;
            const int first_ac = ss == 0 ? 1 : ss;
            unsigned m_lo = 0, m_hi = 0;
            uint32_t first = 0;
            if (valid) {
                if (se > 0) {
                    unsigned long long m = FULL ? m_all : m_all & (~0ull << first_ac) & (~0ull >> (63 - se));
                    m |= zrl_markers(m, first_ac);
                    m_lo = __brev((unsigned)m);
                    m_hi = __brev((unsigned)(m >> 32));
                }
                if (ss == 0) {
                    int size;
                    uint32_t bits;
                    value_code(dcdiff, size, bits);
                    const uint2 e = dc_tab[tbl * 16 + size];
                    first = e.x | bits | e.y << 27;
                }
            }
            *visit_meta(tid) = make_uint4(m_lo, m_hi, first, (unsigned)tbl | (valid ? 0x100u : 0u));
            if (se > 0) {
                const int nnz = __popc(m_lo) + __popc(m_hi);
                const unsigned rank = atomicAdd(&bin[nnz], 1u);
                __syncthreads();
                {
                    const unsigned a = bin[2 * lane], c = bin[2 * lane + 1];
                    unsigned inc = a + c;
#pragma unroll
                    for (int d = 1; d < 32; d <<= 1) {
                        const unsigned o = __shfl_up_sync(0xffffffffu, inc, d);
                        if (lane >= d) inc += o;
                    }
                    const unsigned even = inc - a - c, odd = inc - c;
                    const unsigned e = __shfl_sync(0xffffffffu, even, nnz >> 1), o = __shfl_sync(0xffffffffu, odd, nnz >> 1);
                    order[((nnz & 1) ? o : e) + rank] = (uint16_t)tid;
                }
                __syncthreads();
                for (int i = tid; i < 64; i += T) bin[i] = 0;
            } else {
                order[tid] = (uint16_t)tid;
                __syncthreads();
            }

            if (j == 0) {
                const ItemInfo &nx = items[(round & 1) ^ 1];
                if (!nx.done && (unsigned)tid < nx.n_valid)
                    asm volatile("prefetch.global.L2 [%0];" ::"l"(b.coef + (nx.blk0 + tid) * 64));
            }
            {
                const int src = order[tid];
                const uint4 meta = *visit_meta(src);
                const unsigned inf = meta.w;
                unsigned nb = 0;
                if (inf & 0x100u) {
                    const uint32_t dc_code = meta.z;
                    BitSink<T> sink(scratch, src);
                    sink.put(dc_code & kCodeBits, (int)(dc_code >> 27));
                    if (se > 0) code_nonzeros<T>(meta.x, meta.y, first_ac, se, coef + src * kStageStride, ac_tab + (inf & 0xFF) * 256, sink);
                    nb = sink.finish();
                }
                nbv[src] = nb;
            }
            __syncthreads();

            const unsigned myb = nbv[tid];
            const unsigned nw = (myb + 31) >> 5;
            const uint32_t *mine = scratch + tid;
            uint32_t pre[4];
#pragma unroll
            for (int q = 0; q < 4; ++q) pre[q] = __ldcg(mine + q * T);
            unsigned inc = myb;
#pragma unroll
            for (int d = 1; d < 32; d <<= 1) {
                const unsigned o = __shfl_up_sync(0xffffffffu, inc, d);
                if (lane >= d) inc += o;
            }
            unsigned off = inc - myb, total = 0;
#pragma unroll
            for (int w = 0; w < T / 32; ++w) {
                const unsigned sw = __reduce_add_sync(0xffffffffu, nbv[w * 32 + lane]);
                if (w < warp) off += sw;
                total += sw;
            }
            const unsigned total_words = (total + 31) >> 5;
            const unsigned long long ci = it.chunk_index0 + S.chunk_base;
            const unsigned pool_units = (total_words + 3) >> 2;
            unsigned long long pool_at = 0;
            if (tid == 0) {
                if (pool_units) pool_at = atomicAdd(b.status + kStatPoolCursor, (unsigned long long)pool_units);
                b.chunk_bits[ci] = total;
            }
            for (unsigned wb = 0; wb < total_words; wb += L::kAsmWords) {
                const unsigned nwin = total_words - wb < (unsigned)L::kAsmWords ? total_words - wb : (unsigned)L::kAsmWords;
                for (unsigned i = tid * 4; i < nwin; i += T * 4) *reinterpret_cast<uint4 *>(asmbuf + i) = make_uint4(0, 0, 0, 0);
                __syncthreads();
                if (myb) {
                    const unsigned d0 = off >> 5, dl = (off + myb - 1) >> 5, sft = off & 31;
                    auto word = [&](unsigned q) -> uint32_t {
                        if (q >= nw) return 0u;
                        if (q < 4) return q == 0 ? pre[0] : (q == 1 ? pre[1] : (q == 2 ? pre[2] : pre[3]));
                        return __ldcg(mine + q * T);
                    };
                    if (wb == 0 && dl < nwin) {
                        uint32_t prev = pre[0];
                        atomicOr(asmbuf + d0, prev >> sft);
                        unsigned jw = 1;
                        for (unsigned d = d0 + 1; d < dl; ++d, ++jw) {
                            const uint32_t cur = word(jw);
                            asmbuf[d] = __funnelshift_r(cur, prev, sft);
                            prev = cur;
                        }
                        if (dl > d0) atomicOr(asmbuf + dl, __funnelshift_r(word(jw), prev, sft));
                    } else {
                        const unsigned lo = d0 > wb ? d0 : wb, hi = dl < wb + nwin - 1 ? dl : wb + nwin - 1;
                        if (lo <= hi) {
                            unsigned jw = lo - d0;
                            uint32_t prev = jw > 0 ? word(jw - 1) : 0u;
                            for (unsigned d = lo; d <= hi; ++d, ++jw) {
                                const uint32_t cur = word(jw);
                                atomicOr(asmbuf + (d - wb), __funnelshift_r(cur, prev, sft));
                                prev = cur;
                            }
                        }
                    }
                }
                if (tid == 0 && wb == 0) {
                    if (pool_at + pool_units > b.pool_cap) {
                        atomicOr(b.status + kStatFlags, kFlagPool);
                        pool_at = ~0ull;
                    }
                    wsum[8] = (uint32_t)pool_at;
                    wsum[9] = (uint32_t)(pool_at >> 32);
                    b.chunk_pool[ci] = (uint32_t)pool_at;
                }
                __syncthreads();
                const unsigned long long at = ((unsigned long long)wsum[9] << 32) | wsum[8];
                if (at != ~0ull) {
                    uint4 *dst = reinterpret_cast<uint4 *>(b.pool) + at + (wb >> 2);
                    for (unsigned i = tid; i * 4 < nwin; i += T) dst[i] = reinterpret_cast<const uint4 *>(asmbuf)[i];
                }
                if (wb + L::kAsmWords < total_words || !FULL) __syncthreads();
            }
        }
    }
}

__device__ __forceinline__ unsigned lead_len(const EntropyBuffers &b, const DevPlan &P, unsigned long long img, int k,
                                             unsigned seg_in_scan) {
    if (P.scans[k].rst_base + seg_in_scan > 0) return 2;
    if (k > 0) return P.scans[k].sos_len;
    return b.hdr_len[b.huff_per_image ? img : 0];
}

__global__ void __launch_bounds__(256) segment_len_kernel(const __grid_constant__ EntropyBuffers b, const __grid_constant__ DevPlan P, unsigned long long n_segs) {
    const unsigned long long g = (unsigned long long)blockIdx.x * blockDim.x + threadIdx.x;
    if (g >= n_segs) return;
    const unsigned long long img = g / P.segs_per_image;
    const unsigned s = (unsigned)(g - img * P.segs_per_image);
    const int k = find_scan_by_seg(P, s);
    const DevScan &S = P.scans[k];
    const unsigned i = s - S.seg_base;
    const unsigned cps = P.groups[k % P.n_groups].cps;
    const unsigned long long c0 = img * P.chunks_per_image + S.chunk_base + (unsigned long long)i * cps;
    const unsigned long long bits = b.chunk_bitpos[c0 + cps] - b.chunk_bitpos[c0];
    const unsigned tail = (s == P.segs_per_image - 1 && P.has_eoi) ? 2u : 0u;
    const unsigned long long bytes = lead_len(b, P, img, k, i) + ((bits + 7) >> 3) + tail;
    if (bytes > 0xFFFFFFFFull) atomicOr(b.status + kStatFlags, kFlagSegment4G);
    b.seglen[g] = (unsigned)bytes;
}

__device__ __forceinline__ unsigned long long segment_bytes(const EntropyBuffers &b, const DevPlan &P, unsigned long long g) {
    const unsigned long long img = g / P.segs_per_image;
    const unsigned s = (unsigned)(g - img * P.segs_per_image);
    const int k = find_scan_by_seg(P, s);
    const DevScan &S = P.scans[k];
    const unsigned i = s - S.seg_base;
    const unsigned cps = P.groups[k % P.n_groups].cps;
    const unsigned long long c0 = img * P.chunks_per_image + S.chunk_base + (unsigned long long)i * cps;
    const unsigned long long bits = b.chunk_bitpos[c0 + cps] - b.chunk_bitpos[c0];
    const unsigned tail = (s == P.segs_per_image - 1 && P.has_eoi) ? 2u : 0u;
    return lead_len(b, P, img, k, i) + ((bits + 7) >> 3) + tail;
}

__device__ __forceinline__ unsigned long long cta1024_exclusive(unsigned long long v, unsigned long long *sm, unsigned long long &total) {
    const int lane = threadIdx.x & 31, warp = threadIdx.x >> 5;
    unsigned long long inc = v;
#pragma unroll
    for (int d = 1; d < 32; d <<= 1) {
        const unsigned long long o = __shfl_up_sync(0xffffffffu, inc, d);
        if (lane >= d) inc += o;
    }
    if (lane == 31) sm[warp] = inc;
    __syncthreads();
    if (warp == 0) {
        const unsigned long long w = sm[lane];
        unsigned long long winc = w;
#pragma unroll
        for (int d = 1; d < 32; d <<= 1) {
            const unsigned long long o = __shfl_up_sync(0xffffffffu, winc, d);
            if (lane >= d) winc += o;
        }
        sm[lane] = winc - w;
        if (lane == 31) sm[32] = winc;
    }
    __syncthreads();
    const unsigned long long ex = sm[warp] + inc - v;
    total = sm[32];
    __syncthreads();
    return ex;
}

__global__ void __launch_bounds__(1024) positions_kernel(const __grid_constant__ EntropyBuffers b, const __grid_constant__ DevPlan P, unsigned long long n_chunks,
                                                         unsigned long long n_segs, int scan_chunks) {
    __shared__ unsigned long long sm[33];
    unsigned long long carry = 0, total;
    if (scan_chunks) {
        for (unsigned long long base = 0; base < n_chunks; base += 1024) {
            const unsigned long long i = base + threadIdx.x;
            const unsigned long long ex = cta1024_exclusive(i < n_chunks ? b.chunk_bits[i] : 0ull, sm, total);
            if (i < n_chunks) b.chunk_bitpos[i] = carry + ex;
            carry += total;
        }
        if (threadIdx.x == 0) b.chunk_bitpos[n_chunks] = carry;
        __syncthreads();
    }
    carry = 0;
    for (unsigned long long base = 0; base < n_segs; base += 1024) {
        const unsigned long long g = base + threadIdx.x;
        unsigned long long bytes = 0;
        if (g < n_segs) {
            bytes = segment_bytes(b, P, g);
            if (bytes > 0xFFFFFFFFull) atomicOr(b.status + kStatFlags, kFlagSegment4G);
        }
        const unsigned long long ex = cta1024_exclusive(bytes, sm, total);
        if (g < n_segs) b.segpos[g] = carry + ex;
        carry += total;
    }
    if (threadIdx.x == 0) b.segpos[n_segs] = carry;
}

__device__ __forceinline__ unsigned long long stream_bytes(const EntropyBuffers &b) { return b.segpos[b.n_segs_total]; }
__device__ __forceinline__ bool stream_fits(const EntropyBuffers &b) { return stream_bytes(b) <= b.ustream_cap; }

__device__ __forceinline__ void put_raw(const EntropyBuffers &b, unsigned long long pos, uint8_t byte) {
    b.ustream[pos] = byte;
    atomicOr(b.raw_mask + (pos >> 5), 1u << (pos & 31));
}

__global__ void __launch_bounds__(128) segment_lead_kernel(const __grid_constant__ EntropyBuffers b, const __grid_constant__ DevPlan P, unsigned long long n_segs,
                                                           const unsigned wps) {
    const unsigned long long gw = ((unsigned long long)blockIdx.x * blockDim.x + threadIdx.x) >> 5;
    const unsigned long long g = gw / wps;
    const unsigned slice = (unsigned)(gw - g * wps);
    const int lane = threadIdx.x & 31;
    if (blockIdx.x == 0 && threadIdx.x == 0) {
        const unsigned long long bytes = stream_bytes(b);
        b.status[kStatUnstuffed] = bytes;
        if (bytes > b.ustream_cap) atomicOr(b.status + kStatFlags, kFlagStream);
    }
    if (g >= n_segs || !stream_fits(b)) return;
    const unsigned long long img = g / P.segs_per_image;
    const unsigned s = (unsigned)(g - img * P.segs_per_image);
    const int k = find_scan_by_seg(P, s);
    const DevScan &S = P.scans[k];
    const unsigned i = s - S.seg_base;
    const unsigned long long pos = b.segpos[g];
    {
        const bool eoi = s == P.segs_per_image - 1 && P.has_eoi;
        const unsigned cps = P.groups[k % P.n_groups].cps;
        const unsigned long long c0 = img * P.chunks_per_image + S.chunk_base + (unsigned long long)i * cps;
        const unsigned long long bit0 = b.chunk_bitpos[c0];
        const unsigned long long data0 = pos + lead_len(b, P, img, k, i), data1 = b.segpos[g + 1] - (eoi ? 2u : 0u);
        const unsigned per = (cps + wps) / wps;
        const unsigned q1 = (slice + 1) * per < cps + 1 ? (slice + 1) * per : cps + 1;
        for (unsigned q = slice * per + lane; q < q1; q += 32) {
            const unsigned long long pbit = data0 * 8 + (b.chunk_bitpos[c0 + q] - bit0);
            if ((pbit & 31) == 0) continue;
            const unsigned long long w = pbit >> 5;
            const unsigned long long lo = w * 4 > data0 ? w * 4 : data0, hi = w * 4 + 4 < data1 ? w * 4 + 4 : data1;
            if (lo + 4 == hi) reinterpret_cast<uint32_t *>(b.ustream)[w] = 0u;
            else
                for (unsigned long long x = lo; x < hi; ++x) b.ustream[x] = 0;
        }
    }
    if (slice != 0) return;
    if (S.rst_base + i > 0) {
        if (lane == 0) {
            put_raw(b, pos, 0xFF);
            put_raw(b, pos + 1, (uint8_t)(0xD0 + ((S.rst_base + i - 1) & 7)));
        }
    } else if (k > 0) {
        for (unsigned j = lane; j < S.sos_len; j += 32) put_raw(b, pos + j, P.blob[S.sos_off + j]);
    } else {
        const unsigned long long h = b.huff_per_image ? img : 0;
        const unsigned n = b.hdr_len[h];
        const uint8_t *src = b.hdr + h * b.hdr_stride;
#pragma unroll 4
        for (unsigned j = lane; j < n; j += 32) b.ustream[pos + j] = src[j];
        const unsigned long long w0 = pos >> 5, w1 = (pos + n - 1) >> 5;
        for (unsigned long long w = w0 + lane; w <= w1 && n; w += 32) {
            const unsigned long long lo = w * 32 > pos ? w * 32 : pos, hi = (w + 1) * 32 < pos + n ? (w + 1) * 32 : pos + n;
            const unsigned bits = (unsigned)(hi - lo);
            atomicOr(b.raw_mask + w, (bits == 32 ? 0xFFFFFFFFu : ((1u << bits) - 1u)) << (unsigned)(lo & 31));
        }
    }
    if (s == P.segs_per_image - 1 && P.has_eoi && lane == 0) {
        const unsigned long long end = b.segpos[g + 1];
        put_raw(b, end - 2, 0xFF);
        put_raw(b, end - 1, 0xD9);
    }
}

__global__ void __launch_bounds__(256) place_chunks_kernel(const __grid_constant__ EntropyBuffers b, const __grid_constant__ DevPlan P, unsigned long long n_chunks,
                                                           const unsigned per_warp) {
    if (!stream_fits(b) || (b.status[kStatFlags] & kFlagPool)) return;
    const int lane = threadIdx.x & 31;
    const unsigned long long warps = ((unsigned long long)gridDim.x * blockDim.x) >> 5;
    uint32_t *stream = reinterpret_cast<uint32_t *>(b.ustream);
    for (unsigned long long c0 = (((unsigned long long)blockIdx.x * blockDim.x + threadIdx.x) >> 5) * per_warp; c0 < n_chunks; c0 += warps * per_warp) {
        const unsigned long long c = c0 + lane;
        unsigned my_bits = 0, my_pool = 0;
        unsigned long long my_bitpos = 0;
        if ((unsigned)lane < per_warp && c < n_chunks) {
            const unsigned long long img = c / P.chunks_per_image;
            const unsigned r = (unsigned)(c - img * P.chunks_per_image);
            const int k = find_scan_by_chunk(P, r);
            const DevScan &S = P.scans[k];
            const DevGroup &G = P.groups[k % P.n_groups];
            unsigned seg, q;
            divmod(r - S.chunk_base, G.div_cps, seg, q);
            my_bits = b.chunk_bits[c];
            if (my_bits != 0 || q == 0) {
                const unsigned long long seg_first = b.chunk_bitpos[c - q];
                const unsigned long long data_byte = b.segpos[img * P.segs_per_image + S.seg_base + seg] + lead_len(b, P, img, k, seg);
                my_bitpos = data_byte * 8 + (b.chunk_bitpos[c] - seg_first);
                if (my_bits) my_pool = b.chunk_pool[c];
                if (q == 0) {
                    const unsigned long long seg_bits = b.chunk_bitpos[c + G.cps] - seg_first;
                    const unsigned pad = (unsigned)(-(long long)seg_bits) & 7u;
                    if (pad) {
                        const unsigned long long pbit = data_byte * 8 + seg_bits;
                        const unsigned s2 = (unsigned)(pbit & 31);
                        atomicOr(stream + (pbit >> 5), __byte_perm(((1u << pad) - 1u) << (32 - s2 - pad), 0, 0x0123));
                    }
                }
            }
        }
        unsigned todo = __ballot_sync(0xffffffffu, my_bits != 0);
        while (todo) {
            const int who = __ffs(todo) - 1;
            todo &= todo - 1;
            const unsigned bits = __shfl_sync(0xffffffffu, my_bits, who);
            const unsigned long long bitpos = __shfl_sync(0xffffffffu, my_bitpos, who);
            const uint32_t *src = b.pool + (size_t)__shfl_sync(0xffffffffu, my_pool, who) * 4;
            const unsigned sft = (unsigned)(bitpos & 31);
            uint32_t *dst = stream + (bitpos >> 5);
            const unsigned nw = (bits + 31) >> 5, ndw = (sft + bits + 31) >> 5;
            const bool first_owned = sft == 0, last_owned = ((sft + bits) & 31) == 0;
            uint32_t carry = 0;
            for (unsigned base = 0; base < ndw; base += 128) {
                uint32_t cur[4];
#pragma unroll
                for (int u = 0; u < 4; ++u) {
                    const unsigned d = base + 32 * u + lane;
                    cur[u] = d < nw ? __ldg(src + d) : 0u;
                }
#pragma unroll
                for (int u = 0; u < 4; ++u) {
                    const unsigned d = base + 32 * u + lane;
                    uint32_t prev = __shfl_up_sync(0xffffffffu, cur[u], 1);
                    if (lane == 0) prev = carry;
                    carry = __shfl_sync(0xffffffffu, cur[u], 31);
                    if (d < ndw) {
                        const uint32_t val = sft ? __funnelshift_r(cur[u], prev, sft) : cur[u];
                        const uint32_t be = __byte_perm(val, 0, 0x0123);
                        const bool owned = (d > 0 || first_owned) && (d + 1 < ndw || last_owned);
                        if (owned) dst[d] = be;
                        else atomicOr(dst + d, be);
                    }
                }
            }
        }
    }
}

__device__ __forceinline__ uint32_t ff_flags(uint32_t w) {
    const uint32_t x = ~w;
    const uint32_t t = ((x & 0x7F7F7F7Fu) + 0x7F7F7F7Fu) | x;
    return ~t & 0x80808080u;
}
__device__ __forceinline__ unsigned flags_to_nibble(uint32_t z) { return (((z >> 7) * 0x00204081u) >> 21) & 0xFu; }

__device__ __forceinline__ unsigned ff_bits16(const uint4 d, unsigned raw16, unsigned valid) {
    unsigned m = flags_to_nibble(ff_flags(d.x)) | flags_to_nibble(ff_flags(d.y)) << 4 | flags_to_nibble(ff_flags(d.z)) << 8 |
                 flags_to_nibble(ff_flags(d.w)) << 12;
    m &= ~raw16;
    if (valid < 16) m &= (1u << valid) - 1u;
    return m;
}
__device__ __forceinline__ unsigned ff_count16(const uint4 d, unsigned raw16, unsigned valid) {
    if (raw16 == 0 && valid >= 16) return __popc(ff_flags(d.x)) + __popc(ff_flags(d.y)) + __popc(ff_flags(d.z)) + __popc(ff_flags(d.w));
    return __popc(ff_bits16(d, raw16, valid));
}

__global__ void __launch_bounds__(256) count_ff_kernel(const EntropyBuffers b) {
    __shared__ unsigned warp_sums[8];
    const unsigned long long bytes = stream_fits(b) ? stream_bytes(b) : 0ull;
    const unsigned long long base = (unsigned long long)blockIdx.x * kStuffChunk + (unsigned long long)threadIdx.x * 16;
    unsigned cnt = 0;
    if (base < bytes) {
        const uint4 d = *reinterpret_cast<const uint4 *>(b.ustream + base);
        const unsigned raw = (b.raw_mask[base >> 5] >> (base & 31)) & 0xFFFFu;
        const unsigned valid = bytes - base < 16 ? (unsigned)(bytes - base) : 16u;
        cnt = ff_count16(d, raw, valid);
    }
    cnt = __reduce_add_sync(0xffffffffu, cnt);
    if ((threadIdx.x & 31) == 0) warp_sums[threadIdx.x >> 5] = cnt;
    __syncthreads();
    if (threadIdx.x == 0) {
        unsigned t = 0;
        for (int i = 0; i < 8; ++i) t += warp_sums[i];
        b.ffcount[blockIdx.x] = t;
    }
}

constexpr unsigned kDirectPieces = 2048;

__device__ __forceinline__ void ff_sums_warp(const uint32_t *ffcount, unsigned n_pieces, unsigned idx, int lane, unsigned long long &before, unsigned long long &total) {
    unsigned a = 0, t = 0;
    for (unsigned j = lane; j < n_pieces; j += 32) {
        const unsigned v = ffcount[j];
        t += v;
        if (j < idx) a += v;
    }
    before = __reduce_add_sync(0xffffffffu, a);
    total = __reduce_add_sync(0xffffffffu, t);
}

__device__ __forceinline__ unsigned ff_before_in_chunk(const EntropyBuffers &b, unsigned long long pos, int lane) {
    const unsigned long long start = pos / kStuffChunk * kStuffChunk;
    unsigned ff = 0;
    for (unsigned long long i = start + (unsigned long long)lane * 16; i < pos; i += 32 * 16) {
        const uint4 d = *reinterpret_cast<const uint4 *>(b.ustream + i);
        const unsigned raw = (b.raw_mask[i >> 5] >> (i & 31)) & 0xFFFFu;
        const unsigned valid = pos - i < 16 ? (unsigned)(pos - i) : 16u;
        ff += ff_count16(d, raw, valid);
    }
    return __reduce_add_sync(0xffffffffu, ff);
}

__global__ void __launch_bounds__(256) stuff_scatter_kernel(const __grid_constant__ EntropyBuffers b, const __grid_constant__ DevPlan P, unsigned n_pieces,
                                                            unsigned n_images, unsigned long long *piece_offs) {
    if (!stream_fits(b)) return;
    const unsigned long long bytes = stream_bytes(b);
    const bool direct = n_pieces <= kDirectPieces;
    const int lane = threadIdx.x & 31, warp = threadIdx.x >> 5;
    if (blockIdx.x >= n_pieces) {
        const unsigned k = (blockIdx.x - n_pieces) * 8 + warp;
        const unsigned n_pos = n_images + 1 + (piece_offs ? (unsigned)P.n_scans + 1 : 0u);
        if (k >= n_pos) return;
        unsigned long long pos;
        unsigned long long *dst;
        if (k <= n_images) {
            pos = k == n_images ? bytes : b.segpos[(unsigned long long)k * P.segs_per_image];
            dst = b.file_off + k;
        } else {
            const unsigned sc = k - (n_images + 1);
            pos = sc == (unsigned)P.n_scans ? bytes : b.segpos[P.scans[sc].seg_base];
            dst = piece_offs + sc;
        }
        const unsigned long long piece = pos / kStuffChunk;
        unsigned long long before, total;
        if (direct) ff_sums_warp(b.ffcount, n_pieces, (unsigned)piece, lane, before, total);
        else before = b.ffpos[piece];
        const unsigned ff = ff_before_in_chunk(b, pos, lane);
        if (lane == 0) *dst = pos + before + ff;
        return;
    }
    __shared__ unsigned warp_excl[9];
    __shared__ unsigned long long ff_sm[2];
    __shared__ __align__(16) uint8_t stage[2 * kStuffChunk + 32];
    unsigned long long ff_before, ff_total;
    if (direct) {
        if (warp == 0) {
            unsigned long long a, t;
            ff_sums_warp(b.ffcount, n_pieces, blockIdx.x, lane, a, t);
            if (lane == 0) ff_sm[0] = a, ff_sm[1] = t;
        }
        __syncthreads();
        ff_before = ff_sm[0];
        ff_total = ff_sm[1];
    } else {
        ff_before = b.ffpos[blockIdx.x];
        ff_total = b.ffpos[n_pieces];
    }
    if (blockIdx.x == 0 && threadIdx.x == 0) {
        b.status[kStatDataFF] = ff_total;
        if (bytes + ff_total > b.out_cap) atomicOr(b.status + kStatFlags, kFlagOut);
    }
    if (bytes + ff_total > b.out_cap) return;
    if ((unsigned long long)blockIdx.x * kStuffChunk >= bytes) return;
    const unsigned long long base = (unsigned long long)blockIdx.x * kStuffChunk + (unsigned long long)threadIdx.x * 16;
    uint4 d = make_uint4(0, 0, 0, 0);
    unsigned m = 0, valid = 0;
    if (base < bytes) {
        d = *reinterpret_cast<const uint4 *>(b.ustream + base);
        const unsigned raw = (b.raw_mask[base >> 5] >> (base & 31)) & 0xFFFFu;
        valid = bytes - base < 16 ? (unsigned)(bytes - base) : 16u;
        m = ff_bits16(d, raw, valid);
    }
    const unsigned cnt = __popc(m);
    unsigned inc = cnt;
#pragma unroll
    for (int o = 1; o < 32; o <<= 1) {
        const unsigned t = __shfl_up_sync(0xffffffffu, inc, o);
        if (lane >= o) inc += t;
    }
    if (lane == 31) warp_excl[warp + 1] = inc;
    __syncthreads();
    if (threadIdx.x == 0) {
        warp_excl[0] = 0;
        for (int i = 1; i <= 8; ++i) warp_excl[i] += warp_excl[i - 1];
    }
    __syncthreads();
    const unsigned long long chunk_base = (unsigned long long)blockIdx.x * kStuffChunk;
    const unsigned long long out0 = chunk_base + ff_before;
    const unsigned pad = (unsigned)(out0 & 15);
    const unsigned chunk_in = bytes - chunk_base < kStuffChunk ? (unsigned)(bytes - chunk_base) : (unsigned)kStuffChunk;
    const unsigned total = chunk_in + warp_excl[8];
    if (valid) {
        unsigned o = pad + threadIdx.x * 16 + warp_excl[warp] + (inc - cnt);
        const uint32_t w[4] = {d.x, d.y, d.z, d.w};
#pragma unroll
        for (int i = 0; i < 16; ++i) {
            if ((unsigned)i < valid) {
                stage[o++] = (uint8_t)(w[i >> 2] >> ((i & 3) * 8));
                if (m & (1u << i)) stage[o++] = 0x00;
            }
        }
    }
    __syncthreads();
    uint8_t *dst = b.out + (out0 - pad);
    const unsigned end = pad + total;
    for (unsigned o = threadIdx.x * 16; o < end; o += 256 * 16) {
        if (o >= pad && o + 16 <= end) {
            *reinterpret_cast<uint4 *>(dst + o) = *reinterpret_cast<const uint4 *>(stage + o);
        } else {
            for (unsigned k = (o < pad ? pad : o); k < o + 16 && k < end; ++k) dst[k] = stage[k];
        }
    }
}

template <int BASE>
__device__ __forceinline__ void count_half(unsigned m, int &next, unsigned c_shared, unsigned *ha) {
#pragma unroll 1
    while (m) {
        int p;
        asm("bfind.u32 %0, %1;" : "=r"(p) : "r"(m));
        unsigned bit;
        asm("bmsk.clamp.b32 %0, %1, 1;" : "=r"(bit) : "r"(p));
        m ^= bit;
        const int k = BASE + 31 - p;
        int v;
        asm("ld.shared.s16 %0, [%1];" : "=r"(v) : "r"(c_shared + 2 * k));
        const int run = k - next;
        next = k + 1;
        const int a = v < 0 ? -v : v;
        int top;
        asm("bfind.u32 %0, %1;" : "=r"(top) : "r"(a));
        atomicAdd(ha + ((run << 4) | (top + 1)), 1u);
    }
}

__global__ void __launch_bounds__(256) histogram_kernel(const __grid_constant__ DevPlan P, const int16_t *coef, unsigned n_images, uint32_t *hist,
                                                        int bands, int per_band) {
    __shared__ unsigned sh[2 * 2 * 257];
    __shared__ __align__(16) int16_t blk[256 * kStageStride];
    const int tid = threadIdx.x;
    const unsigned long long g0 = (unsigned long long)blockIdx.x * 256;
    const unsigned n_here = P.blocks_per_image - g0 < 256 ? (unsigned)(P.blocks_per_image - g0) : 256u;
    for (unsigned img = blockIdx.y; img < n_images; img += gridDim.y) {
        for (int i = tid; i < 2 * 2 * 257; i += 256) sh[i] = 0;
        const int16_t *src = coef + ((unsigned long long)img * P.blocks_per_image + g0) * 64;
        {
            const unsigned pieces = n_here * 8;
            const char *g = reinterpret_cast<const char *>(src) + (size_t)tid * 16;
            const unsigned d = (unsigned)__cvta_generic_to_shared(blk) + (tid >> 3) * (kStageStride * 2) + (tid & 7) * 16;
#pragma unroll
            for (int k = 0; k < 8; ++k)
                if ((unsigned)(tid + k * 256) < pieces)
                    asm volatile("cp.async.cg.shared.global [%0], [%1], 16;" ::"r"(d + k * 32 * (kStageStride * 2)), "l"(g + k * 256 * 16) : "memory");
            asm volatile("cp.async.wait_all;" ::: "memory");
        }
        __syncthreads();
        if ((unsigned)tid < n_here) {
            const unsigned long long g = g0 + tid;
            int comp = 0;
            while (comp + 1 < P.n_groups && g >= P.groups[comp + 1].block_base) ++comp;
            const int16_t *mine = blk + tid * kStageStride;
            const uint4 *m4 = reinterpret_cast<const uint4 *>(mine);
            unsigned m_lo = 0, m_hi = 0;
#pragma unroll
            for (int w = 0; w < 8; ++w) {
                const uint4 q = m4[w];
                unsigned byte = __dp2a_lo(nonzero16x2(q.x), 0x0201u, 0u);
                byte = __dp2a_lo(nonzero16x2(q.y), 0x0804u, byte);
                byte = __dp2a_lo(nonzero16x2(q.z), 0x2010u, byte);
                byte = __dp2a_lo(nonzero16x2(q.w), 0x8040u, byte);
                if (w < 4) m_lo |= byte << (8 * w);
                else m_hi |= byte << (8 * (w - 4));
            }
            const unsigned long long m_all = (((unsigned long long)m_hi << 32) | m_lo) & ~1ull;
            const int prev = g > P.groups[comp].block_base ? (tid > 0 ? (int)mine[-kStageStride] : (int)__ldg(src - 64)) : 0;
            unsigned *h = sh + P.comp_tbl[comp] * 2 * 257;
            const int diff = (int)(int16_t)(mine[0] - prev);
            atomicAdd(h + (32 - __clz(diff < 0 ? -diff : diff)), 1u);
            unsigned *ha = h + 257;
            const unsigned c_shared = (unsigned)__cvta_generic_to_shared(mine);
            for (int b = 0; b < bands; ++b) {
                const int first_ac = b == 0 ? 1 : b * per_band, se = b == bands - 1 ? 63 : (b + 1) * per_band - 1;
                if (se < first_ac) continue;
                unsigned long long m = m_all & (~0ull << first_ac) & (~0ull >> (63 - se));
                m |= zrl_markers(m, first_ac);
                int next = first_ac;
                count_half<0>(__brev((unsigned)m), next, c_shared, ha);
                count_half<32>(__brev((unsigned)(m >> 32)), next, c_shared, ha);
                if (next <= se) atomicAdd(ha, 1u);
            }
        }
        __syncthreads();
        uint32_t *dst = hist + (size_t)img * (2 * 2 * 257);
        for (int i = tid; i < 2 * 2 * 257; i += 256)
            if (sh[i]) atomicAdd(dst + i, sh[i]);
        __syncthreads();
    }
}

}

static inline unsigned grid_for(unsigned long long n, unsigned block) { return (unsigned)((n + block - 1) / block); }

cudaError_t launch_histogram(const DevPlan &hp, const int16_t *coef, uint32_t n_images, uint32_t *hist,
                             cudaStream_t stream) {
    const int bands = hp.spg > 1 ? hp.spg - 1 : 1;
    const int per_band = bands > 1 ? 64 / bands : 64;
    dim3 grid(grid_for(hp.blocks_per_image, 256), n_images < 32768 ? n_images : 32768);
    histogram_kernel<<<grid, 256, 0, stream>>>(hp, coef, n_images, hist, bands, per_band);
    return cudaGetLastError();
}

namespace {
template <int T, bool FULL>
cudaError_t coder_config(unsigned long long n_items, CoderLaunch &cfg) {
    unsigned long long grid = 0;
    cudaError_t e = resident_ctas<encode_chunks_kernel<T, FULL>>(T, CoderSmem<T, FULL>::kBytes, grid);
    if (e != cudaSuccess) return e;
    if (grid > n_items) grid = n_items;
    if (grid < 1) grid = 1;
    cfg.grid = (unsigned)grid;
    cfg.smem = CoderSmem<T, FULL>::kBytes;
    cfg.scratch_bytes = (size_t)grid * T * kSlotWords * 4;
    return cudaSuccess;
}
inline bool plan_is_full(const DevPlan &hp) { return hp.scans[hp.n_scans - 1].ss == 0 && hp.scans[hp.n_scans - 1].se == 63; }
}

#define JPGB_CODER_DISPATCH(CALL)                              \
    do {                                                       \
        const bool full = plan_is_full(hp);                    \
        switch (hp.chunk_T) {                                  \
        case 32: if (full) { CALL(32, true); } else { CALL(32, false); } break;    \
        case 64: if (full) { CALL(64, true); } else { CALL(64, false); } break;    \
        case 128: if (full) { CALL(128, true); } else { CALL(128, false); } break; \
        default: if (full) { CALL(256, true); } else { CALL(256, false); } break;  \
        }                                                      \
    } while (0)

cudaError_t coder_launch_config(const DevPlan &hp, uint32_t n, CoderLaunch &cfg) {
    const unsigned long long n_items = (unsigned long long)hp.items_per_image * n;
#define JPGB_CFG(T, F) return coder_config<T, F>(n_items, cfg)
    JPGB_CODER_DISPATCH(JPGB_CFG);
#undef JPGB_CFG
    return cudaErrorInvalidValue;
}
cudaError_t launch_encode_chunks(const EntropyBuffers &b, const DevPlan &hp, uint32_t n, const CoderLaunch &cfg, cudaStream_t s) {
    const unsigned long long n_items = (unsigned long long)hp.items_per_image * n;
#define JPGB_RUN(T, F) encode_chunks_kernel<T, F><<<cfg.grid, T, cfg.smem, s>>>(b, hp, n_items)
    JPGB_CODER_DISPATCH(JPGB_RUN);
#undef JPGB_RUN
    return cudaGetLastError();
}
cudaError_t launch_segment_lengths(const EntropyBuffers &b, const DevPlan &hp, uint32_t n, cudaStream_t s) {
    const unsigned long long ns = (unsigned long long)hp.segs_per_image * n;
    segment_len_kernel<<<grid_for(ns, 256), 256, 0, s>>>(b, hp, ns);
    return cudaGetLastError();
}
cudaError_t launch_positions(const EntropyBuffers &b, const DevPlan &hp, uint32_t n, bool scan_chunks, cudaStream_t s) {
    positions_kernel<<<1, 1024, 0, s>>>(b, hp, (unsigned long long)hp.chunks_per_image * n, (unsigned long long)hp.segs_per_image * n, scan_chunks ? 1 : 0);
    return cudaGetLastError();
}
cudaError_t launch_segment_leads(const EntropyBuffers &b, const DevPlan &hp, uint32_t n, cudaStream_t s) {
    const unsigned long long ns = (unsigned long long)hp.segs_per_image * n;
    unsigned cps = 1;
    for (int g = 0; g < hp.n_groups; ++g) cps = hp.groups[g].cps > cps ? hp.groups[g].cps : cps;
    unsigned wps = (cps + 1 + 127) / 128;
    wps = wps > 1024 ? 1024 : wps;
    segment_lead_kernel<<<grid_for(ns * wps * 32, 128), 128, 0, s>>>(b, hp, ns, wps);
    return cudaGetLastError();
}
cudaError_t launch_place_chunks(const EntropyBuffers &b, const DevPlan &hp, uint32_t n, cudaStream_t s) {
    const unsigned long long nc = (unsigned long long)hp.chunks_per_image * n;
    unsigned per_warp = 1;
    while (per_warp < 32 && nc / (per_warp * 2) >= 16384) per_warp *= 2;
    const unsigned long long ctas = (nc + 8ull * per_warp - 1) / (8ull * per_warp);
    place_chunks_kernel<<<(unsigned)(ctas < 65536 ? (ctas ? ctas : 1) : 65536), 256, 0, s>>>(b, hp, nc, per_warp);
    return cudaGetLastError();
}
cudaError_t launch_count_ff(const EntropyBuffers &b, cudaStream_t s) {
    count_ff_kernel<<<grid_for(b.ustream_cap, kStuffChunk), 256, 0, s>>>(b);
    return cudaGetLastError();
}
bool ff_scan_needed(const EntropyBuffers &b) { return grid_for(b.ustream_cap, kStuffChunk) > kDirectPieces; }
cudaError_t launch_stuff_scatter(const EntropyBuffers &b, const DevPlan &hp, uint32_t n, unsigned long long *piece_offs, cudaStream_t s) {
    const unsigned n_pieces = grid_for(b.ustream_cap, kStuffChunk);
    const unsigned n_pos = n + 1 + (piece_offs ? (unsigned)hp.n_scans + 1 : 0u);
    stuff_scatter_kernel<<<n_pieces + (n_pos + 7) / 8, 256, 0, s>>>(b, hp, n_pieces, n, piece_offs);
    return cudaGetLastError();
}

}
```

jpeg_encoder_b200/csrc/kernels.h:

```cpp
#pragma once
#include <cuda_runtime.h>

#include <cstdint>
#include <mutex>

#include "../../include/jpegenc_b200.h"
#include "device_types.h"

namespace jpgb {

template <auto Kernel>
cudaError_t resident_ctas(int threads, size_t smem, unsigned long long &ctas) {
    constexpr int kMaxDevices = 64;
    static std::mutex mu;
    static struct {
        int dev = -1;
        unsigned long long ctas = 0;
    } cache[kMaxDevices];
    int dev = 0;
    cudaGetDevice(&dev);
    std::lock_guard<std::mutex> lock(mu);
    auto &c = cache[dev < kMaxDevices ? dev : kMaxDevices - 1];
    if (c.dev != dev) {
        cudaError_t e = cudaFuncSetAttribute(Kernel, cudaFuncAttributeMaxDynamicSharedMemorySize, (int)smem);
        if (e != cudaSuccess) return e;
        int n_sms = 0, per_sm = 0;
        cudaDeviceGetAttribute(&n_sms, cudaDevAttrMultiProcessorCount, dev);
        e = cudaOccupancyMaxActiveBlocksPerMultiprocessor(&per_sm, Kernel, threads, smem);
        if (e != cudaSuccess) return e;
        c.ctas = (unsigned long long)n_sms * (per_sm < 1 ? 1 : per_sm);
        c.dev = dev;
    }
    ctas = c.ctas;
    return cudaSuccess;
}

cudaError_t launch_stage_a(const StageAParams &p, uint32_t n_images, cudaStream_t stream);

constexpr size_t kHuffWordsPerImage = 2 * 2 * 256;

struct EntropyBuffers {
    const int16_t *coef;
    const uint32_t *huff;
    int huff_per_image;
    uint32_t *scratch;
    uint32_t *pool;
    unsigned long long pool_cap;
    uint32_t *chunk_bits;
    uint32_t *chunk_pool;
    unsigned long long *chunk_bitpos;
    uint32_t *seglen;
    unsigned long long *segpos;
    const uint32_t *hdr_len;
    const uint8_t *hdr;
    uint32_t hdr_stride;
    uint8_t *ustream;
    uint32_t *raw_mask;
    uint32_t *ffcount;
    unsigned long long *ffpos;
    uint8_t *out;
    unsigned long long *file_off;
    void *scan_tmp;
    unsigned long long ustream_cap, out_cap, n_segs_total;
    unsigned long long *status;
    size_t scan_tmp_bytes;
};

constexpr int kStatusWords = 8;
constexpr int kStatUnstuffed = 0, kStatDataFF = 1, kStatFlags = 2, kStatScanError = 3, kStatTicket = 4, kStatPoolCursor = 5;
constexpr unsigned long long kFlagStream = 1, kFlagOut = 2, kFlagPool = 4, kFlagSegment4G = 8, kFlagHuffmanLong = 16;

struct StatusBlock {
    uint32_t n;
    size_t mask_bytes;
    size_t readback_bytes() const { return (size_t)(n + 1 + 2 * kStatusWords) * 8; }
    size_t bytes() const { return readback_bytes() + mask_bytes; }
    unsigned long long *file_off(void *base) const { return static_cast<unsigned long long *>(base); }
    unsigned long long *status(void *base) const { return file_off(base) + n + 1; }
    unsigned long long *table_status(void *base) const { return status(base) + kStatusWords; }
    uint32_t *raw_mask(void *base) const { return reinterpret_cast<uint32_t *>(table_status(base) + kStatusWords); }
};
inline StatusBlock status_block(uint32_t n, unsigned long long ustream_cap) { return {n, (size_t)(ustream_cap / 32 + 2) * 4}; }

constexpr int kSlotWords = 56;
constexpr int kStuffChunk = 4096;

cudaError_t launch_histogram(const DevPlan &hplan, const int16_t *coef, uint32_t n_images,
                             uint32_t *hist , cudaStream_t stream);
struct CoderLaunch {
    unsigned grid;
    size_t smem, scratch_bytes;
};
cudaError_t coder_launch_config(const DevPlan &hplan, uint32_t n_images, CoderLaunch &cfg);
cudaError_t launch_encode_chunks(const EntropyBuffers &b, const DevPlan &hplan, uint32_t n_images, const CoderLaunch &cfg, cudaStream_t stream);
cudaError_t launch_segment_lengths(const EntropyBuffers &b, const DevPlan &hplan, uint32_t n_images, cudaStream_t stream);
cudaError_t launch_positions(const EntropyBuffers &b, const DevPlan &hplan, uint32_t n_images, bool scan_chunks, cudaStream_t stream);
cudaError_t launch_segment_leads(const EntropyBuffers &b, const DevPlan &hplan, uint32_t n_images, cudaStream_t stream);
cudaError_t launch_place_chunks(const EntropyBuffers &b, const DevPlan &hplan, uint32_t n_images, cudaStream_t stream);
cudaError_t launch_count_ff(const EntropyBuffers &b, cudaStream_t stream);
bool ff_scan_needed(const EntropyBuffers &b);
cudaError_t launch_stuff_scatter(const EntropyBuffers &b, const DevPlan &hplan, uint32_t n_images, unsigned long long *piece_offs, cudaStream_t stream);

cudaError_t launch_build_tables(const uint32_t *hist, int hist_per_image, int n_tables, uint32_t n_images, uint32_t *huff, const uint8_t *head,
                                uint32_t head_len, const uint8_t *tail, uint32_t tail_len, uint8_t *hdr, uint32_t hdr_stride, uint32_t *hdr_len,
                                unsigned long long *status, cudaStream_t stream);

cudaError_t launch_build_single_tables(const uint32_t *hist, uint32_t n, int ac, uint32_t *words, uint8_t *dht, uint32_t *dht_len, uint32_t *bad,
                                       cudaStream_t stream);

cudaError_t launch_place_pieces(const uint8_t *src, uint8_t *dst, unsigned long long dst_cap, const unsigned long long *table, unsigned world,
                                unsigned rank, unsigned n_scans, unsigned long long *total_out, cudaStream_t stream);

size_t scan_tmp_bytes(uint64_t n);
cudaError_t launch_exclusive_scan(const uint32_t *in, unsigned long long *out, uint64_t n, void *tmp, cudaStream_t stream,
                                  uint32_t *launches, unsigned long long *err_flag = nullptr);

}
```

Measured before the change: 309,400.

## Compose stuffed pieces directly from chunk pool instead of materializing unstuffed stream

Replaces the segment-lead, chunk-placement, FF-count and stuff-scatter kernels with two piece kernels. Each CTA locates the segments and chunks overlapping its 4 KiB piece with a cooperative search, then composes 16-byte groups straight from the chunk pool and header/marker bytes. This drops the intermediate unstuffed stream buffer, the raw-byte mask with its atomics, and the clear and poison memsets on that buffer. In exchange the composition work runs twice, once to count FF bytes and once to stuff them, and the per-piece binary searches and shared-memory tables add their own cost.

```diff
diff --git a/jpeg_encoder_b200/csrc/api.cu b/jpeg_encoder_b200/csrc/api.cu
--- a/jpeg_encoder_b200/csrc/api.cu
+++ b/jpeg_encoder_b200/csrc/api.cu
@@ -101,7 +101,7 @@
 
 struct GraphKey {
     PlanSig sig;
-    uint64_t words[39];
+    uint64_t words[38];
 };
 
 struct GraphCache {
@@ -158,7 +158,7 @@
     cudaStream_t stream = nullptr;
     bool own_stream = false;
     std::string err;
-    DevBuf pixels, coef, huff, hdr, hdr_len, scratch, pool, chunk_bits, chunk_pool, chunk_bitpos, seglen, segpos, ustream, ffcount, ffpos,
+    DevBuf pixels, coef, huff, hdr, hdr_len, scratch, pool, chunk_bits, chunk_pool, chunk_bitpos, seglen, segpos, piece_start, ffcount, ffpos,
         out, scan_tmp, hist, piece_off, out2, pixels2, status, hdr_parts;
     std::vector<uint8_t> last_tables;
     double ucap_ratio = 0;
@@ -429,14 +429,9 @@
                      const HeaderLayout &hl, const SequenceFlags &f) {
     cudaStream_t st = enc->stream;
     const uint64_t n_chunks = (uint64_t)plan.chunks_per_image * n, n_segs = b.n_segs_total, n_pieces = b.ustream_cap / kStuffChunk;
-    const StatusBlock sb = status_block(n, b.ustream_cap);
+    const StatusBlock sb = status_block(n);
     unsigned long long *scan_err = b.status + kStatScanError;
-    if (f.coder) {
-        CK(cudaMemsetAsync(b.status, 0, 2 * kStatusWords * 8 + sb.mask_bytes, st), "clear status and raw mask");
-    } else {
-        CK(cudaMemsetAsync(b.status, 0, (kStatScanError + 1) * 8, st), "clear status");
-        CK(cudaMemsetAsync(b.raw_mask, 0, sb.mask_bytes, st), "clear raw mask");
-    }
+    CK(cudaMemsetAsync(b.status, 0, f.coder ? 2 * kStatusWords * 8 : (kStatScanError + 1) * 8, st), "clear status");
     if (f.tables) {
         StageTimer t(enc, 1);
         if (!f.given_hist) {
@@ -468,17 +463,15 @@
     }
     {
         StageTimer t(enc, 3);
-        if (f.poison) CK(cudaMemsetAsync(b.ustream, 0xFF, b.ustream_cap + 64, st), "poison stream");
-        CK(launch_segment_leads(b, hp, n, st), "segment lead launch");
-        CK(launch_place_chunks(b, hp, n, st), "placement launch");
-        enc->launches += 2;
+        CK(launch_count_pieces(b, hp, n, st), "piece count launch");
+        enc->launches += 1;
     }
     {
         StageTimer t(enc, 4);
-        CK(launch_count_ff(b, st), "count ff launch");
         if (ff_scan_needed(b)) CK(launch_exclusive_scan(b.ffcount, b.ffpos, n_pieces, b.scan_tmp, st, &enc->launches, scan_err), "ff scan");
-        CK(launch_stuff_scatter(b, hp, n, f.pieces ? enc->piece_off.as<unsigned long long>() : nullptr, st), "scatter launch");
-        enc->launches += 2;
+        if (f.poison) CK(cudaMemsetAsync(b.out, 0xFF, b.out_cap + 64, st), "poison output");
+        CK(launch_stuff_pieces(b, hp, n, f.pieces ? enc->piece_off.as<unsigned long long>() : nullptr, st), "stuffing launch");
+        enc->launches += 1;
         if (f.pieces)
             CK(cudaMemcpyAsync(enc->h_pieces.p, enc->piece_off.p, (plan.scans.size() + 1) * 8, cudaMemcpyDeviceToHost, st), "read piece offsets");
         CK(cudaMemcpyAsync(enc->h_small.p, b.file_off, sb.readback_bytes(), cudaMemcpyDeviceToHost, st), "read file offsets and status");
@@ -488,11 +481,11 @@
 
 GraphKey graph_key(const jpgb_encoder *enc, const PlanSig &sig, const EntropyBuffers &b, uint32_t n, const CoderLaunch &coder,
                    const HeaderLayout &hl, const SequenceFlags &f) {
-    static_assert(sizeof(EntropyBuffers) == 26 * 8, "every field of EntropyBuffers takes part in the graph key");
+    static_assert(sizeof(EntropyBuffers) == 25 * 8, "every field of EntropyBuffers takes part in the graph key");
     GraphKey k{{}, {
         (uint64_t)b.coef, (uint64_t)b.huff, (uint64_t)b.huff_per_image, (uint64_t)b.scratch, (uint64_t)b.pool, b.pool_cap,
         (uint64_t)b.chunk_bits, (uint64_t)b.chunk_pool, (uint64_t)b.chunk_bitpos, (uint64_t)b.seglen, (uint64_t)b.segpos,
-        (uint64_t)b.hdr_len, (uint64_t)b.hdr, b.hdr_stride, (uint64_t)b.ustream, (uint64_t)b.raw_mask, (uint64_t)b.ffcount,
+        (uint64_t)b.hdr_len, (uint64_t)b.hdr, b.hdr_stride, (uint64_t)b.piece_start, (uint64_t)b.ffcount,
         (uint64_t)b.ffpos, (uint64_t)b.out, (uint64_t)b.file_off, (uint64_t)b.scan_tmp, b.ustream_cap, b.out_cap, b.n_segs_total,
         (uint64_t)b.status, b.scan_tmp_bytes,
         coder.grid, coder.smem, coder.scratch_bytes, n,
@@ -561,7 +554,7 @@
     CoderLaunch coder{};
     CK(coder_launch_config(hp, n, coder), "coder configuration");
     CK(enc->scratch.reserve(coder.scratch_bytes), "alloc coder scratch");
-    CK(enc->h_small.reserve(status_block(n, 0).readback_bytes()), "alloc readback");
+    CK(enc->h_small.reserve(status_block(n).readback_bytes()), "alloc readback");
     if (piece_offsets) {
         CK(enc->piece_off.reserve((plan.scans.size() + 1) * 8), "alloc piece offsets");
         CK(enc->h_pieces.reserve((plan.scans.size() + 1) * 8), "alloc piece offsets (host)");
@@ -594,9 +587,9 @@
     for (int attempt = 0;; ++attempt) {
         caps.ustream = (caps.ustream + kStuffChunk - 1) / kStuffChunk * kStuffChunk;
         const uint64_t n_pieces = caps.ustream / kStuffChunk;
-        const StatusBlock sb = status_block(n, caps.ustream);
-        CK(enc->ustream.reserve(caps.ustream + 64), "alloc unstuffed stream");
-        CK(enc->status.reserve(sb.bytes()), "alloc status and raw mask");
+        const StatusBlock sb = status_block(n);
+        CK(enc->piece_start.reserve(n_pieces * 16), "alloc piece starts");
+        CK(enc->status.reserve(sb.bytes()), "alloc status");
         CK(enc->ffcount.reserve((n_pieces + 1) * 4), "alloc ff counts");
         CK(enc->ffpos.reserve((n_pieces + 2) * 8), "alloc ff positions");
         CK(enc->scan_tmp.reserve(scan_tmp_bytes(std::max<uint64_t>(n_pieces, std::max(n_chunks, n_segs)))), "alloc scan scratch");
@@ -604,10 +597,9 @@
         CK(out.reserve(caps.out + 64), "alloc output");
         b.pool = enc->pool.as<uint32_t>();
         b.pool_cap = caps.pool_units;
-        b.ustream = enc->ustream.as<uint8_t>();
+        b.piece_start = enc->piece_start.as<unsigned long long>();
         b.file_off = sb.file_off(enc->status.p);
         b.status = sb.status(enc->status.p);
-        b.raw_mask = sb.raw_mask(enc->status.p);
         b.ffcount = enc->ffcount.as<uint32_t>();
         b.ffpos = enc->ffpos.as<unsigned long long>();
         b.scan_tmp = enc->scan_tmp.p;
diff --git a/jpeg_encoder_b200/csrc/entropy.cu b/jpeg_encoder_b200/csrc/entropy.cu
--- a/jpeg_encoder_b200/csrc/entropy.cu
+++ b/jpeg_encoder_b200/csrc/entropy.cu
@@ -1,5 +1,6 @@
 
 #include "kernels.h"
+#include "piece_compose.h"
 
 namespace jpgb {
 namespace {
@@ -521,185 +522,179 @@
 __device__ __forceinline__ unsigned long long stream_bytes(const EntropyBuffers &b) { return b.segpos[b.n_segs_total]; }
 __device__ __forceinline__ bool stream_fits(const EntropyBuffers &b) { return stream_bytes(b) <= b.ustream_cap; }
 
-__device__ __forceinline__ void put_raw(const EntropyBuffers &b, unsigned long long pos, uint8_t byte) {
-    b.ustream[pos] = byte;
-    atomicOr(b.raw_mask + (pos >> 5), 1u << (pos & 31));
-}
-
-__global__ void __launch_bounds__(128) segment_lead_kernel(const __grid_constant__ EntropyBuffers b, const __grid_constant__ DevPlan P, unsigned long long n_segs,
-                                                           const unsigned wps) {
-    const unsigned long long gw = ((unsigned long long)blockIdx.x * blockDim.x + threadIdx.x) >> 5;
-    const unsigned long long g = gw / wps;
-    const unsigned slice = (unsigned)(gw - g * wps);
-    const int lane = threadIdx.x & 31;
-    if (blockIdx.x == 0 && threadIdx.x == 0) {
-        const unsigned long long bytes = stream_bytes(b);
+constexpr int kPieceThreads = 128;
+constexpr int kGroupsPerThread = kStuffChunk / 16 / kPieceThreads;
+constexpr int kPieceMinCtas = 12;
+
+struct SegGeom {
+    unsigned long long img, c0;
+    int k;
+    unsigned i, cps;
+};
+__device__ __forceinline__ SegGeom seg_geom(const DevPlan &P, unsigned long long g) {
+    SegGeom r;
+    r.img = g / P.segs_per_image;
+    const unsigned s = (unsigned)(g - r.img * P.segs_per_image);
+    r.k = find_scan_by_seg(P, s);
+    r.i = s - P.scans[r.k].seg_base;
+    r.cps = P.groups[r.k % P.n_groups].cps;
+    r.c0 = r.img * P.chunks_per_image + P.scans[r.k].chunk_base + (unsigned long long)r.i * r.cps;
+    return r;
+}
+
+struct DevLayout {
+    const EntropyBuffers &b;
+    const DevPlan &P;
+    __device__ unsigned long long n_segs() const { return b.n_segs_total; }
+    __device__ unsigned long long seg_lo(unsigned long long g) const { return b.segpos[g]; }
+    __device__ unsigned long long seg_chunk0(unsigned long long g) const { return seg_geom(P, g).c0; }
+    __device__ unsigned long long seg_cps(unsigned long long g) const { return seg_geom(P, g).cps; }
+    __device__ unsigned long long seg_data0(unsigned long long g) const {
+        const SegGeom s = seg_geom(P, g);
+        return b.segpos[g] + lead_len(b, P, s.img, s.k, s.i);
+    }
+    __device__ unsigned long long chunk_pos(unsigned long long c) const { return b.chunk_bitpos[c]; }
+};
+
+__device__ __forceinline__ piece::SegRun make_seg_run(const EntropyBuffers &b, const DevPlan &P, unsigned long long g) {
+    const SegGeom s = seg_geom(P, g);
+    const DevScan &S = P.scans[s.k];
+    piece::SegRun r;
+    r.lo = b.segpos[g];
+    r.hi = b.segpos[g + 1];
+    r.mark = 0;
+    r.spare = 0;
+    unsigned len;
+    if (S.rst_base + s.i > 0) {
+        r.lead = nullptr;
+        r.mark = 0xFFu | (0xD0u + ((S.rst_base + s.i - 1) & 7)) << 8;
+        len = 2;
+    } else if (s.k > 0) {
+        r.lead = P.blob + S.sos_off;
+        len = S.sos_len;
+    } else {
+        const unsigned long long h = b.huff_per_image ? s.img : 0;
+        r.lead = b.hdr + h * b.hdr_stride;
+        len = b.hdr_len[h];
+    }
+    r.d0 = r.lo + len;
+    r.pbit = r.d0 * 8 + (b.chunk_bitpos[s.c0 + s.cps] - b.chunk_bitpos[s.c0]);
+    return r;
+}
+
+__device__ __forceinline__ piece::ChunkRun make_chunk_run(const EntropyBuffers &b, const DevPlan &P, unsigned long long c) {
+    const unsigned long long img = c / P.chunks_per_image;
+    const unsigned r = (unsigned)(c - img * P.chunks_per_image);
+    const int k = find_scan_by_chunk(P, r);
+    const DevScan &S = P.scans[k];
+    unsigned seg, q;
+    divmod(r - S.chunk_base, P.groups[k % P.n_groups].div_cps, seg, q);
+    const unsigned long long data0 = b.segpos[img * P.segs_per_image + S.seg_base + seg] + lead_len(b, P, img, k, seg);
+    piece::ChunkRun cr;
+    cr.bit0 = data0 * 8 + (b.chunk_bitpos[c] - b.chunk_bitpos[c - q]);
+    cr.bits = b.chunk_bits[c];
+    cr.src = b.pool + (size_t)b.chunk_pool[c] * 4;
+    cr.spare = 0;
+    return cr;
+}
+
+struct PieceTables {
+    piece::SegRun seg[kPieceThreads];
+    piece::ChunkRun ch[kPieceThreads];
+};
+
+struct CtaSearch {
+    template <class Key>
+    __device__ unsigned long long operator()(unsigned long long lo, unsigned long long hi, Key key, unsigned long long x) const {
+        while (lo < hi) {
+            const unsigned long long step = (hi - lo + kPieceThreads) / kPieceThreads;
+            const unsigned long long i = lo + step * threadIdx.x;
+            const int n = __syncthreads_count(i <= hi && key(i) <= x);
+            lo += step * (unsigned long long)(n - 1);
+            hi = lo + step - 1 < hi ? lo + step - 1 : hi;
+        }
+        return lo;
+    }
+};
+
+__device__ __forceinline__ void compose_piece(const EntropyBuffers &b, const DevPlan &P, unsigned long long n_chunks, unsigned long long g,
+                                              unsigned long long c, unsigned long long x0, unsigned long long x1, PieceTables &t,
+                                              uint32_t (&w)[kGroupsPerThread][4], unsigned (&raw)[kGroupsPerThread]) {
+    __shared__ unsigned long long first_base;
+    const int tid = threadIdx.x;
+#pragma unroll
+    for (int j = 0; j < kGroupsPerThread; ++j) {
+        w[j][0] = w[j][1] = w[j][2] = w[j][3] = 0;
+        raw[j] = 0;
+    }
+    for (;;) {
+        const bool has_s = g + tid < b.n_segs_total, has_c = c + tid < n_chunks;
+        const unsigned long long sp = has_s ? b.segpos[g + tid] : 0ull, cb = has_c ? b.chunk_bitpos[c + tid] : 0ull;
+        if (tid == 0 && has_c) {
+            t.ch[0] = make_chunk_run(b, P, c);
+            first_base = t.ch[0].bit0 - cb;
+        }
+        __syncthreads();
+        const bool seg_in = has_s && sp < x1;
+        bool ch_in = false;
+        if (seg_in) t.seg[tid] = make_seg_run(b, P, g + tid);
+        if (tid == 0) ch_in = has_c && t.ch[0].bit0 < x1 * 8;
+        else if (has_c && first_base + cb < x1 * 8) {
+            const piece::ChunkRun r = make_chunk_run(b, P, c + tid);
+            ch_in = r.bit0 < x1 * 8;
+            if (ch_in) t.ch[tid] = r;
+        }
+        const int ns = __syncthreads_count(seg_in), nc = __syncthreads_count(ch_in);
+#pragma unroll
+        for (int j = 0; j < kGroupsPerThread; ++j) {
+            const unsigned long long x = x0 + 16ull * (tid + j * kPieceThreads);
+            if (x < x1) piece::compose16(t.seg, ns, t.ch, nc, x, w[j], raw[j]);
+        }
+        if (ns < kPieceThreads && nc < kPieceThreads) break;
+        g += ns;
+        c += nc;
+        __syncthreads();
+    }
+}
+
+__global__ void __launch_bounds__(kPieceThreads, kPieceMinCtas) count_pieces_kernel(const __grid_constant__ EntropyBuffers b, const __grid_constant__ DevPlan P,
+                                                                     unsigned long long n_chunks) {
+    __shared__ PieceTables t;
+    __shared__ unsigned warp_sums[kPieceThreads / 32];
+    const unsigned long long bytes = stream_bytes(b);
+    const unsigned p = blockIdx.x;
+    if (p == 0 && threadIdx.x == 0) {
         b.status[kStatUnstuffed] = bytes;
         if (bytes > b.ustream_cap) atomicOr(b.status + kStatFlags, kFlagStream);
     }
-    if (g >= n_segs || !stream_fits(b)) return;
-    const unsigned long long img = g / P.segs_per_image;
-    const unsigned s = (unsigned)(g - img * P.segs_per_image);
-    const int k = find_scan_by_seg(P, s);
-    const DevScan &S = P.scans[k];
-    const unsigned i = s - S.seg_base;
-    const unsigned long long pos = b.segpos[g];
-    {
-        const bool eoi = s == P.segs_per_image - 1 && P.has_eoi;
-        const unsigned cps = P.groups[k % P.n_groups].cps;
-        const unsigned long long c0 = img * P.chunks_per_image + S.chunk_base + (unsigned long long)i * cps;
-        const unsigned long long bit0 = b.chunk_bitpos[c0];
-        const unsigned long long data0 = pos + lead_len(b, P, img, k, i), data1 = b.segpos[g + 1] - (eoi ? 2u : 0u);
-        const unsigned per = (cps + wps) / wps;
-        const unsigned q1 = (slice + 1) * per < cps + 1 ? (slice + 1) * per : cps + 1;
-        for (unsigned q = slice * per + lane; q < q1; q += 32) {
-            const unsigned long long pbit = data0 * 8 + (b.chunk_bitpos[c0 + q] - bit0);
-            if ((pbit & 31) == 0) continue;
-            const unsigned long long w = pbit >> 5;
-            const unsigned long long lo = w * 4 > data0 ? w * 4 : data0, hi = w * 4 + 4 < data1 ? w * 4 + 4 : data1;
-            if (lo + 4 == hi) reinterpret_cast<uint32_t *>(b.ustream)[w] = 0u;
-            else
-                for (unsigned long long x = lo; x < hi; ++x) b.ustream[x] = 0;
-        }
-    }
-    if (slice != 0) return;
-    if (S.rst_base + i > 0) {
-        if (lane == 0) {
-            put_raw(b, pos, 0xFF);
-            put_raw(b, pos + 1, (uint8_t)(0xD0 + ((S.rst_base + i - 1) & 7)));
-        }
-    } else if (k > 0) {
-        for (unsigned j = lane; j < S.sos_len; j += 32) put_raw(b, pos + j, P.blob[S.sos_off + j]);
-    } else {
-        const unsigned long long h = b.huff_per_image ? img : 0;
-        const unsigned n = b.hdr_len[h];
-        const uint8_t *src = b.hdr + h * b.hdr_stride;
-#pragma unroll 4
-        for (unsigned j = lane; j < n; j += 32) b.ustream[pos + j] = src[j];
-        const unsigned long long w0 = pos >> 5, w1 = (pos + n - 1) >> 5;
-        for (unsigned long long w = w0 + lane; w <= w1 && n; w += 32) {
-            const unsigned long long lo = w * 32 > pos ? w * 32 : pos, hi = (w + 1) * 32 < pos + n ? (w + 1) * 32 : pos + n;
-            const unsigned bits = (unsigned)(hi - lo);
-            atomicOr(b.raw_mask + w, (bits == 32 ? 0xFFFFFFFFu : ((1u << bits) - 1u)) << (unsigned)(lo & 31));
-        }
-    }
-    if (s == P.segs_per_image - 1 && P.has_eoi && lane == 0) {
-        const unsigned long long end = b.segpos[g + 1];
-        put_raw(b, end - 2, 0xFF);
-        put_raw(b, end - 1, 0xD9);
-    }
-}
-
-__global__ void __launch_bounds__(256) place_chunks_kernel(const __grid_constant__ EntropyBuffers b, const __grid_constant__ DevPlan P, unsigned long long n_chunks,
-                                                           const unsigned per_warp) {
-    if (!stream_fits(b) || (b.status[kStatFlags] & kFlagPool)) return;
-    const int lane = threadIdx.x & 31;
-    const unsigned long long warps = ((unsigned long long)gridDim.x * blockDim.x) >> 5;
-    uint32_t *stream = reinterpret_cast<uint32_t *>(b.ustream);
-    for (unsigned long long c0 = (((unsigned long long)blockIdx.x * blockDim.x + threadIdx.x) >> 5) * per_warp; c0 < n_chunks; c0 += warps * per_warp) {
-        const unsigned long long c = c0 + lane;
-        unsigned my_bits = 0, my_pool = 0;
-        unsigned long long my_bitpos = 0;
-        if ((unsigned)lane < per_warp && c < n_chunks) {
-            const unsigned long long img = c / P.chunks_per_image;
-            const unsigned r = (unsigned)(c - img * P.chunks_per_image);
-            const int k = find_scan_by_chunk(P, r);
-            const DevScan &S = P.scans[k];
-            const DevGroup &G = P.groups[k % P.n_groups];
-            unsigned seg, q;
-            divmod(r - S.chunk_base, G.div_cps, seg, q);
-            my_bits = b.chunk_bits[c];
-            if (my_bits != 0 || q == 0) {
-                const unsigned long long seg_first = b.chunk_bitpos[c - q];
-                const unsigned long long data_byte = b.segpos[img * P.segs_per_image + S.seg_base + seg] + lead_len(b, P, img, k, seg);
-                my_bitpos = data_byte * 8 + (b.chunk_bitpos[c] - seg_first);
-                if (my_bits) my_pool = b.chunk_pool[c];
-                if (q == 0) {
-                    const unsigned long long seg_bits = b.chunk_bitpos[c + G.cps] - seg_first;
-                    const unsigned pad = (unsigned)(-(long long)seg_bits) & 7u;
-                    if (pad) {
-                        const unsigned long long pbit = data_byte * 8 + seg_bits;
-                        const unsigned s2 = (unsigned)(pbit & 31);
-                        atomicOr(stream + (pbit >> 5), __byte_perm(((1u << pad) - 1u) << (32 - s2 - pad), 0, 0x0123));
-                    }
-                }
-            }
-        }
-        unsigned todo = __ballot_sync(0xffffffffu, my_bits != 0);
-        while (todo) {
-            const int who = __ffs(todo) - 1;
-            todo &= todo - 1;
-            const unsigned bits = __shfl_sync(0xffffffffu, my_bits, who);
-            const unsigned long long bitpos = __shfl_sync(0xffffffffu, my_bitpos, who);
-            const uint32_t *src = b.pool + (size_t)__shfl_sync(0xffffffffu, my_pool, who) * 4;
-            const unsigned sft = (unsigned)(bitpos & 31);
-            uint32_t *dst = stream + (bitpos >> 5);
-            const unsigned nw = (bits + 31) >> 5, ndw = (sft + bits + 31) >> 5;
-            const bool first_owned = sft == 0, last_owned = ((sft + bits) & 31) == 0;
-            uint32_t carry = 0;
-            for (unsigned base = 0; base < ndw; base += 128) {
-                uint32_t cur[4];
-#pragma unroll
-                for (int u = 0; u < 4; ++u) {
-                    const unsigned d = base + 32 * u + lane;
-                    cur[u] = d < nw ? __ldg(src + d) : 0u;
-                }
-#pragma unroll
-                for (int u = 0; u < 4; ++u) {
-                    const unsigned d = base + 32 * u + lane;
-                    uint32_t prev = __shfl_up_sync(0xffffffffu, cur[u], 1);
-                    if (lane == 0) prev = carry;
-                    carry = __shfl_sync(0xffffffffu, cur[u], 31);
-                    if (d < ndw) {
-                        const uint32_t val = sft ? __funnelshift_r(cur[u], prev, sft) : cur[u];
-                        const uint32_t be = __byte_perm(val, 0, 0x0123);
-                        const bool owned = (d > 0 || first_owned) && (d + 1 < ndw || last_owned);
-                        if (owned) dst[d] = be;
-                        else atomicOr(dst + d, be);
-                    }
-                }
-            }
-        }
-    }
-}
-
-__device__ __forceinline__ uint32_t ff_flags(uint32_t w) {
-    const uint32_t x = ~w;
-    const uint32_t t = ((x & 0x7F7F7F7Fu) + 0x7F7F7F7Fu) | x;
-    return ~t & 0x80808080u;
-}
-__device__ __forceinline__ unsigned flags_to_nibble(uint32_t z) { return (((z >> 7) * 0x00204081u) >> 21) & 0xFu; }
-
-__device__ __forceinline__ unsigned ff_bits16(const uint4 d, unsigned raw16, unsigned valid) {
-    unsigned m = flags_to_nibble(ff_flags(d.x)) | flags_to_nibble(ff_flags(d.y)) << 4 | flags_to_nibble(ff_flags(d.z)) << 8 |
-                 flags_to_nibble(ff_flags(d.w)) << 12;
-    m &= ~raw16;
-    if (valid < 16) m &= (1u << valid) - 1u;
-    return m;
-}
-__device__ __forceinline__ unsigned ff_count16(const uint4 d, unsigned raw16, unsigned valid) {
-    if (raw16 == 0 && valid >= 16) return __popc(ff_flags(d.x)) + __popc(ff_flags(d.y)) + __popc(ff_flags(d.z)) + __popc(ff_flags(d.w));
-    return __popc(ff_bits16(d, raw16, valid));
-}
-
-__global__ void __launch_bounds__(256) count_ff_kernel(const EntropyBuffers b) {
-    __shared__ unsigned warp_sums[8];
-    const unsigned long long bytes = stream_fits(b) ? stream_bytes(b) : 0ull;
-    const unsigned long long base = (unsigned long long)blockIdx.x * kStuffChunk + (unsigned long long)threadIdx.x * 16;
+    const unsigned long long x0 = (unsigned long long)p * kStuffChunk;
+    if (bytes > b.ustream_cap || (b.status[kStatFlags] & kFlagPool) || x0 >= bytes) {
+        if (threadIdx.x == 0) b.ffcount[p] = 0;
+        return;
+    }
+    const unsigned long long x1 = bytes - x0 < kStuffChunk ? bytes : x0 + kStuffChunk;
+    unsigned long long g, c;
+    piece::find_piece_start(DevLayout{b, P}, x0, g, c, CtaSearch());
+    if (threadIdx.x == 0) {
+        b.piece_start[2ull * p] = g;
+        b.piece_start[2ull * p + 1] = c;
+    }
+    uint32_t w[kGroupsPerThread][4];
+    unsigned raw[kGroupsPerThread];
+    compose_piece(b, P, n_chunks, g, c, x0, x1, t, w, raw);
     unsigned cnt = 0;
-    if (base < bytes) {
-        const uint4 d = *reinterpret_cast<const uint4 *>(b.ustream + base);
-        const unsigned raw = (b.raw_mask[base >> 5] >> (base & 31)) & 0xFFFFu;
-        const unsigned valid = bytes - base < 16 ? (unsigned)(bytes - base) : 16u;
-        cnt = ff_count16(d, raw, valid);
+#pragma unroll
+    for (int j = 0; j < kGroupsPerThread; ++j) {
+        uint32_t le[4];
+        cnt += __popc(piece::data_ff16(w[j], raw[j], le));
     }
     cnt = __reduce_add_sync(0xffffffffu, cnt);
     if ((threadIdx.x & 31) == 0) warp_sums[threadIdx.x >> 5] = cnt;
     __syncthreads();
     if (threadIdx.x == 0) {
-        unsigned t = 0;
-        for (int i = 0; i < 8; ++i) t += warp_sums[i];
-        b.ffcount[blockIdx.x] = t;
+        unsigned s = 0;
+        for (int i = 0; i < kPieceThreads / 32; ++i) s += warp_sums[i];
+        b.ffcount[p] = s;
     }
 }
 
@@ -716,117 +711,151 @@
     total = __reduce_add_sync(0xffffffffu, t);
 }
 
-__device__ __forceinline__ unsigned ff_before_in_chunk(const EntropyBuffers &b, unsigned long long pos, int lane) {
-    const unsigned long long start = pos / kStuffChunk * kStuffChunk;
-    unsigned ff = 0;
-    for (unsigned long long i = start + (unsigned long long)lane * 16; i < pos; i += 32 * 16) {
-        const uint4 d = *reinterpret_cast<const uint4 *>(b.ustream + i);
-        const unsigned raw = (b.raw_mask[i >> 5] >> (i & 31)) & 0xFFFFu;
-        const unsigned valid = pos - i < 16 ? (unsigned)(pos - i) : 16u;
-        ff += ff_count16(d, raw, valid);
-    }
-    return __reduce_add_sync(0xffffffffu, ff);
-}
-
-__global__ void __launch_bounds__(256) stuff_scatter_kernel(const __grid_constant__ EntropyBuffers b, const __grid_constant__ DevPlan P, unsigned n_pieces,
-                                                            unsigned n_images, unsigned long long *piece_offs) {
-    if (!stream_fits(b)) return;
-    const unsigned long long bytes = stream_bytes(b);
-    const bool direct = n_pieces <= kDirectPieces;
-    const int lane = threadIdx.x & 31, warp = threadIdx.x >> 5;
-    if (blockIdx.x >= n_pieces) {
-        const unsigned k = (blockIdx.x - n_pieces) * 8 + warp;
-        const unsigned n_pos = n_images + 1 + (piece_offs ? (unsigned)P.n_scans + 1 : 0u);
-        if (k >= n_pos) return;
-        unsigned long long pos;
-        unsigned long long *dst;
-        if (k <= n_images) {
-            pos = k == n_images ? bytes : b.segpos[(unsigned long long)k * P.segs_per_image];
-            dst = b.file_off + k;
-        } else {
-            const unsigned sc = k - (n_images + 1);
-            pos = sc == (unsigned)P.n_scans ? bytes : b.segpos[P.scans[sc].seg_base];
-            dst = piece_offs + sc;
-        }
-        const unsigned long long piece = pos / kStuffChunk;
-        unsigned long long before, total;
-        if (direct) ff_sums_warp(b.ffcount, n_pieces, (unsigned)piece, lane, before, total);
-        else before = b.ffpos[piece];
-        const unsigned ff = ff_before_in_chunk(b, pos, lane);
-        if (lane == 0) *dst = pos + before + ff;
-        return;
-    }
-    __shared__ unsigned warp_excl[9];
+__global__ void __launch_bounds__(kPieceThreads, kPieceMinCtas) stuff_pieces_kernel(const __grid_constant__ EntropyBuffers b, const __grid_constant__ DevPlan P,
+                                                                     unsigned long long n_chunks, unsigned n_pieces, unsigned n_images,
+                                                                     unsigned long long *piece_offs) {
+    __shared__ PieceTables t;
+    __shared__ __align__(16) uint32_t tile[kStuffChunk / 4 + 4];
+    __shared__ uint32_t ffw[kStuffChunk / 32 + 2];
+    __shared__ uint16_t gstart[kStuffChunk / 16];
+    __shared__ unsigned scan_sm[kPieceThreads / 32];
     __shared__ unsigned long long ff_sm[2];
-    __shared__ __align__(16) uint8_t stage[2 * kStuffChunk + 32];
+    const unsigned p = blockIdx.x;
+    const unsigned long long bytes = stream_bytes(b), flags = b.status[kStatFlags];
+    const unsigned long long g0 = p < b.ustream_cap / kStuffChunk ? b.piece_start[2ull * p] : 0ull;
+    const unsigned long long c0 = p < b.ustream_cap / kStuffChunk ? b.piece_start[2ull * p + 1] : 0ull;
+    if (bytes > b.ustream_cap || (flags & kFlagPool)) return;
+    const int tid = threadIdx.x, lane = tid & 31, warp = tid >> 5;
     unsigned long long ff_before, ff_total;
-    if (direct) {
+    if (n_pieces <= kDirectPieces) {
         if (warp == 0) {
-            unsigned long long a, t;
-            ff_sums_warp(b.ffcount, n_pieces, blockIdx.x, lane, a, t);
-            if (lane == 0) ff_sm[0] = a, ff_sm[1] = t;
+            unsigned long long a, s;
+            ff_sums_warp(b.ffcount, n_pieces, p, lane, a, s);
+            if (lane == 0) ff_sm[0] = a, ff_sm[1] = s;
         }
         __syncthreads();
         ff_before = ff_sm[0];
         ff_total = ff_sm[1];
     } else {
-        ff_before = b.ffpos[blockIdx.x];
+        ff_before = b.ffpos[p];
         ff_total = b.ffpos[n_pieces];
     }
-    if (blockIdx.x == 0 && threadIdx.x == 0) {
+    const unsigned long long out_bytes = bytes + ff_total;
+    if (p == 0 && tid == 0) {
         b.status[kStatDataFF] = ff_total;
-        if (bytes + ff_total > b.out_cap) atomicOr(b.status + kStatFlags, kFlagOut);
-    }
-    if (bytes + ff_total > b.out_cap) return;
-    if ((unsigned long long)blockIdx.x * kStuffChunk >= bytes) return;
-    const unsigned long long base = (unsigned long long)blockIdx.x * kStuffChunk + (unsigned long long)threadIdx.x * 16;
-    uint4 d = make_uint4(0, 0, 0, 0);
-    unsigned m = 0, valid = 0;
-    if (base < bytes) {
-        d = *reinterpret_cast<const uint4 *>(b.ustream + base);
-        const unsigned raw = (b.raw_mask[base >> 5] >> (base & 31)) & 0xFFFFu;
-        valid = bytes - base < 16 ? (unsigned)(bytes - base) : 16u;
-        m = ff_bits16(d, raw, valid);
-    }
-    const unsigned cnt = __popc(m);
-    unsigned inc = cnt;
-#pragma unroll
-    for (int o = 1; o < 32; o <<= 1) {
-        const unsigned t = __shfl_up_sync(0xffffffffu, inc, o);
-        if (lane >= o) inc += t;
-    }
-    if (lane == 31) warp_excl[warp + 1] = inc;
+        if (out_bytes > b.out_cap) atomicOr(b.status + kStatFlags, kFlagOut);
+        b.file_off[n_images] = out_bytes;
+        if (piece_offs) piece_offs[P.n_scans] = out_bytes;
+    }
+    if (out_bytes > b.out_cap) return;
+    const unsigned long long x0 = (unsigned long long)p * kStuffChunk;
+    if (x0 >= bytes) return;
+    const unsigned long long x1 = bytes - x0 < kStuffChunk ? bytes : x0 + kStuffChunk;
+
+    uint32_t w[kGroupsPerThread][4];
+    unsigned raw[kGroupsPerThread];
+    compose_piece(b, P, n_chunks, g0, c0, x0, x1, t, w, raw);
+    unsigned m[kGroupsPerThread], packed = 0;
+#pragma unroll
+    for (int j = 0; j < kGroupsPerThread; ++j) {
+        uint32_t le[4];
+        m[j] = piece::data_ff16(w[j], raw[j], le);
+        const int grp = tid + j * kPieceThreads;
+        reinterpret_cast<uint4 *>(tile)[grp] = make_uint4(le[0], le[1], le[2], le[3]);
+        reinterpret_cast<uint16_t *>(ffw)[grp] = (uint16_t)m[j];
+        packed |= (unsigned)__popc(m[j]) << (16 * j);
+    }
+    if (tid < 8) tile[kStuffChunk / 4 + (tid & 3)] = 0, ffw[kStuffChunk / 32 + (tid & 1)] = 0;
+    unsigned inc = packed;
+#pragma unroll
+    for (int d = 1; d < 32; d <<= 1) {
+        const unsigned o = __shfl_up_sync(0xffffffffu, inc, d);
+        if (lane >= d) inc += o;
+    }
+    if (lane == 31) scan_sm[warp] = inc;
     __syncthreads();
-    if (threadIdx.x == 0) {
-        warp_excl[0] = 0;
-        for (int i = 1; i <= 8; ++i) warp_excl[i] += warp_excl[i - 1];
-    }
+    unsigned before = 0, all = 0;
+#pragma unroll
+    for (int i = 0; i < kPieceThreads / 32; ++i) {
+        const unsigned v = scan_sm[i];
+        if (i < warp) before += v;
+        all += v;
+    }
+    const unsigned ex = before + inc - packed;
+    static_assert(kGroupsPerThread == 2, "the scan packs two groups per thread");
+    gstart[tid] = (uint16_t)(16 * tid + (ex & 0xFFFFu));
+    gstart[tid + kPieceThreads] = (uint16_t)(16 * (tid + kPieceThreads) + (all & 0xFFFFu) + (ex >> 16));
+    const unsigned ff_piece = (all & 0xFFFFu) + (all >> 16);
     __syncthreads();
-    const unsigned long long chunk_base = (unsigned long long)blockIdx.x * kStuffChunk;
-    const unsigned long long out0 = chunk_base + ff_before;
+
+    const unsigned chunk_in = (unsigned)(x1 - x0);
+    const unsigned total = chunk_in + ff_piece;
+    const unsigned long long out0 = x0 + ff_before;
     const unsigned pad = (unsigned)(out0 & 15);
-    const unsigned chunk_in = bytes - chunk_base < kStuffChunk ? (unsigned)(bytes - chunk_base) : (unsigned)kStuffChunk;
-    const unsigned total = chunk_in + warp_excl[8];
-    if (valid) {
-        unsigned o = pad + threadIdx.x * 16 + warp_excl[warp] + (inc - cnt);
-        const uint32_t w[4] = {d.x, d.y, d.z, d.w};
-#pragma unroll
-        for (int i = 0; i < 16; ++i) {
-            if ((unsigned)i < valid) {
-                stage[o++] = (uint8_t)(w[i >> 2] >> ((i & 3) * 8));
-                if (m & (1u << i)) stage[o++] = 0x00;
-            }
-        }
-    }
-    __syncthreads();
-    uint8_t *dst = b.out + (out0 - pad);
-    const unsigned end = pad + total;
-    for (unsigned o = threadIdx.x * 16; o < end; o += 256 * 16) {
-        if (o >= pad && o + 16 <= end) {
-            *reinterpret_cast<uint4 *>(dst + o) = *reinterpret_cast<const uint4 *>(stage + o);
-        } else {
-            for (unsigned k = (o < pad ? pad : o); k < o + 16 && k < end; ++k) dst[k] = stage[k];
-        }
+    uint8_t *const dst = b.out + (out0 - pad);
+    auto is_ff = [&](unsigned i) { return (ffw[i >> 5] >> (i & 31)) & 1u; };
+    auto in_byte = [&](unsigned i) { return (uint32_t)reinterpret_cast<const uint8_t *>(tile)[i]; };
+    auto group_of = [&](unsigned y) {
+        unsigned lo = 0, hi = kStuffChunk / 16 - 1;
+        while (lo < hi) {
+            const unsigned mid = (lo + hi + 1) >> 1;
+            if (gstart[mid] <= y) lo = mid;
+            else hi = mid - 1;
+        }
+        return lo;
+    };
+    const unsigned n_blk = (pad + total + 15) >> 4;
+    for (unsigned q = tid; q < n_blk; q += kPieceThreads) {
+        const int y = (int)(16 * q) - (int)pad;
+        const bool full = y >= 0 && y + 16 <= (int)total;
+        const unsigned y0 = y < 0 ? 0u : (unsigned)y;
+        const unsigned g = group_of(y0);
+        const unsigned yr = y0 - gstart[g];
+        const unsigned mg = reinterpret_cast<const uint16_t *>(ffw)[g];
+        if (full && mg == 0) {
+            const unsigned i0 = 16 * g + yr;
+            const unsigned long long pair = (unsigned long long)ffw[(i0 >> 5) + 1] << 32 | ffw[i0 >> 5];
+            if (((pair >> (i0 & 31)) & 0x7FFFu) == 0) {
+                const uint32_t *s = tile + (i0 >> 2);
+                const unsigned sh = (i0 & 3) * 8;
+                const uint32_t a0 = s[0], a1 = s[1], a2 = s[2], a3 = s[3], a4 = s[4];
+                *reinterpret_cast<uint4 *>(dst + 16 * q) = make_uint4(__funnelshift_r(a0, a1, sh), __funnelshift_r(a1, a2, sh),
+                                                                      __funnelshift_r(a2, a3, sh), __funnelshift_r(a3, a4, sh));
+                continue;
+            }
+        }
+        unsigned j = 0, at = 0;
+        while (at + 1 + ((mg >> j) & 1u) <= yr) at += 1 + ((mg >> j) & 1u), ++j;
+        unsigned i = 16 * g + j;
+        bool zero = at != yr;
+        uint32_t v[4] = {0, 0, 0, 0};
+#pragma unroll
+        for (int k = 0; k < 16; ++k) {
+            const int yk = y + k;
+            if (yk >= (int)y0 && yk < (int)total) {
+                const uint32_t byte = zero ? 0u : in_byte(i);
+                if (full) v[k >> 2] |= byte << (8 * (k & 3));
+                else dst[16 * q + k] = (uint8_t)byte;
+                if (!zero && is_ff(i)) zero = true;
+                else zero = false, ++i;
+            }
+        }
+        if (full) *reinterpret_cast<uint4 *>(dst + 16 * q) = make_uint4(v[0], v[1], v[2], v[3]);
+    }
+
+    for (unsigned long long g = g0 + tid; g < b.n_segs_total; g += kPieceThreads) {
+        const unsigned long long lo = b.segpos[g];
+        if (lo >= x1) break;
+        if (lo < x0) continue;
+        const unsigned long long img = g / P.segs_per_image;
+        const unsigned s = (unsigned)(g - img * P.segs_per_image);
+        const bool scan_first = piece_offs && img == 0 && P.scans[find_scan_by_seg(P, s)].seg_base == s;
+        if (s != 0 && !scan_first) continue;
+        const unsigned i = (unsigned)(lo - x0), gi = i >> 4;
+        const unsigned ff = gstart[gi] - 16 * gi + __popc(reinterpret_cast<const uint16_t *>(ffw)[gi] & ((1u << (i & 15)) - 1u));
+        const unsigned long long at = lo + ff_before + ff;
+        if (s == 0) b.file_off[img] = at;
+        if (scan_first) piece_offs[find_scan_by_seg(P, s)] = at;
     }
 }
 
@@ -978,33 +1007,15 @@
     positions_kernel<<<1, 1024, 0, s>>>(b, hp, (unsigned long long)hp.chunks_per_image * n, (unsigned long long)hp.segs_per_image * n, scan_chunks ? 1 : 0);
     return cudaGetLastError();
 }
-cudaError_t launch_segment_leads(const EntropyBuffers &b, const DevPlan &hp, uint32_t n, cudaStream_t s) {
-    const unsigned long long ns = (unsigned long long)hp.segs_per_image * n;
-    unsigned cps = 1;
-    for (int g = 0; g < hp.n_groups; ++g) cps = hp.groups[g].cps > cps ? hp.groups[g].cps : cps;
-    unsigned wps = (cps + 1 + 127) / 128;
-    wps = wps > 1024 ? 1024 : wps;
-    segment_lead_kernel<<<grid_for(ns * wps * 32, 128), 128, 0, s>>>(b, hp, ns, wps);
+cudaError_t launch_count_pieces(const EntropyBuffers &b, const DevPlan &hp, uint32_t n, cudaStream_t s) {
+    count_pieces_kernel<<<grid_for(b.ustream_cap, kStuffChunk), kPieceThreads, 0, s>>>(b, hp, (unsigned long long)hp.chunks_per_image * n);
     return cudaGetLastError();
 }
-cudaError_t launch_place_chunks(const EntropyBuffers &b, const DevPlan &hp, uint32_t n, cudaStream_t s) {
-    const unsigned long long nc = (unsigned long long)hp.chunks_per_image * n;
-    unsigned per_warp = 1;
-    while (per_warp < 32 && nc / (per_warp * 2) >= 16384) per_warp *= 2;
-    const unsigned long long ctas = (nc + 8ull * per_warp - 1) / (8ull * per_warp);
-    place_chunks_kernel<<<(unsigned)(ctas < 65536 ? (ctas ? ctas : 1) : 65536), 256, 0, s>>>(b, hp, nc, per_warp);
+bool ff_scan_needed(const EntropyBuffers &b) { return grid_for(b.ustream_cap, kStuffChunk) > kDirectPieces; }
+cudaError_t launch_stuff_pieces(const EntropyBuffers &b, const DevPlan &hp, uint32_t n, unsigned long long *piece_offs, cudaStream_t s) {
+    const unsigned n_pieces = grid_for(b.ustream_cap, kStuffChunk);
+    stuff_pieces_kernel<<<n_pieces, kPieceThreads, 0, s>>>(b, hp, (unsigned long long)hp.chunks_per_image * n, n_pieces, n, piece_offs);
     return cudaGetLastError();
 }
-cudaError_t launch_count_ff(const EntropyBuffers &b, cudaStream_t s) {
-    count_ff_kernel<<<grid_for(b.ustream_cap, kStuffChunk), 256, 0, s>>>(b);
-    return cudaGetLastError();
-}
-bool ff_scan_needed(const EntropyBuffers &b) { return grid_for(b.ustream_cap, kStuffChunk) > kDirectPieces; }
-cudaError_t launch_stuff_scatter(const EntropyBuffers &b, const DevPlan &hp, uint32_t n, unsigned long long *piece_offs, cudaStream_t s) {
-    const unsigned n_pieces = grid_for(b.ustream_cap, kStuffChunk);
-    const unsigned n_pos = n + 1 + (piece_offs ? (unsigned)hp.n_scans + 1 : 0u);
-    stuff_scatter_kernel<<<n_pieces + (n_pos + 7) / 8, 256, 0, s>>>(b, hp, n_pieces, n, piece_offs);
-    return cudaGetLastError();
-}
-
-}
+
+}
diff --git a/jpeg_encoder_b200/csrc/kernels.h b/jpeg_encoder_b200/csrc/kernels.h
--- a/jpeg_encoder_b200/csrc/kernels.h
+++ b/jpeg_encoder_b200/csrc/kernels.h
@@ -54,8 +54,7 @@
     const uint32_t *hdr_len;
     const uint8_t *hdr;
     uint32_t hdr_stride;
-    uint8_t *ustream;
-    uint32_t *raw_mask;
+    unsigned long long *piece_start;
     uint32_t *ffcount;
     unsigned long long *ffpos;
     uint8_t *out;
@@ -72,15 +71,13 @@
 
 struct StatusBlock {
     uint32_t n;
-    size_t mask_bytes;
     size_t readback_bytes() const { return (size_t)(n + 1 + 2 * kStatusWords) * 8; }
-    size_t bytes() const { return readback_bytes() + mask_bytes; }
+    size_t bytes() const { return readback_bytes(); }
     unsigned long long *file_off(void *base) const { return static_cast<unsigned long long *>(base); }
     unsigned long long *status(void *base) const { return file_off(base) + n + 1; }
     unsigned long long *table_status(void *base) const { return status(base) + kStatusWords; }
-    uint32_t *raw_mask(void *base) const { return reinterpret_cast<uint32_t *>(table_status(base) + kStatusWords); }
 };
-inline StatusBlock status_block(uint32_t n, unsigned long long ustream_cap) { return {n, (size_t)(ustream_cap / 32 + 2) * 4}; }
+inline StatusBlock status_block(uint32_t n) { return {n}; }
 
 constexpr int kSlotWords = 56;
 constexpr int kStuffChunk = 4096;
@@ -95,11 +92,9 @@
 cudaError_t launch_encode_chunks(const EntropyBuffers &b, const DevPlan &hplan, uint32_t n_images, const CoderLaunch &cfg, cudaStream_t stream);
 cudaError_t launch_segment_lengths(const EntropyBuffers &b, const DevPlan &hplan, uint32_t n_images, cudaStream_t stream);
 cudaError_t launch_positions(const EntropyBuffers &b, const DevPlan &hplan, uint32_t n_images, bool scan_chunks, cudaStream_t stream);
-cudaError_t launch_segment_leads(const EntropyBuffers &b, const DevPlan &hplan, uint32_t n_images, cudaStream_t stream);
-cudaError_t launch_place_chunks(const EntropyBuffers &b, const DevPlan &hplan, uint32_t n_images, cudaStream_t stream);
-cudaError_t launch_count_ff(const EntropyBuffers &b, cudaStream_t stream);
+cudaError_t launch_count_pieces(const EntropyBuffers &b, const DevPlan &hplan, uint32_t n_images, cudaStream_t stream);
 bool ff_scan_needed(const EntropyBuffers &b);
-cudaError_t launch_stuff_scatter(const EntropyBuffers &b, const DevPlan &hplan, uint32_t n_images, unsigned long long *piece_offs, cudaStream_t stream);
+cudaError_t launch_stuff_pieces(const EntropyBuffers &b, const DevPlan &hplan, uint32_t n_images, unsigned long long *piece_offs, cudaStream_t stream);
 
 cudaError_t launch_build_tables(const uint32_t *hist, int hist_per_image, int n_tables, uint32_t n_images, uint32_t *huff, const uint8_t *head,
                                 uint32_t head_len, const uint8_t *tail, uint32_t tail_len, uint8_t *hdr, uint32_t hdr_stride, uint32_t *hdr_len,
diff --git a/jpeg_encoder_b200/csrc/piece_compose.h b/jpeg_encoder_b200/csrc/piece_compose.h
--- /dev/null
+++ b/jpeg_encoder_b200/csrc/piece_compose.h
@@ -0,0 +1,155 @@
+#pragma once
+#include <cstdint>
+
+#ifdef __CUDACC__
+#define JPGB_HD __host__ __device__ __forceinline__
+#define JPGB_UNROLL _Pragma("unroll")
+#else
+#define JPGB_HD inline
+#define JPGB_UNROLL
+#endif
+
+namespace jpgb {
+namespace piece {
+
+struct SegRun {
+    unsigned long long lo, d0, pbit, hi;
+    const uint8_t *lead;
+    uint32_t mark, spare;
+};
+struct ChunkRun {
+    unsigned long long bit0;
+    const uint32_t *src;
+    uint32_t bits, spare;
+};
+
+JPGB_HD uint32_t fshl(uint32_t lo, uint32_t hi, unsigned s) {
+#ifdef __CUDA_ARCH__
+    return __funnelshift_l(lo, hi, s);
+#else
+    return s ? (hi << s) | (lo >> (32 - s)) : hi;
+#endif
+}
+JPGB_HD uint32_t bswap(uint32_t w) {
+#ifdef __CUDA_ARCH__
+    return __byte_perm(w, 0, 0x0123);
+#else
+    return __builtin_bswap32(w);
+#endif
+}
+JPGB_HD uint32_t load_pool(const uint32_t *p) {
+#ifdef __CUDA_ARCH__
+    return __ldg(p);
+#else
+    return *p;
+#endif
+}
+
+JPGB_HD void or_byte(uint32_t w[4], unsigned j, uint32_t v) {
+JPGB_UNROLL
+    for (unsigned k = 0; k < 4; ++k)
+        if ((j >> 2) == k) w[k] |= v << (24 - 8 * (j & 3));
+}
+
+template <class End>
+JPGB_HD int first_ending_after(int n, unsigned long long pos, End end) {
+    int lo = 0, hi = n;
+    while (lo < hi) {
+        const int mid = (lo + hi) >> 1;
+        if (end(mid) > pos) hi = mid;
+        else lo = mid + 1;
+    }
+    return lo;
+}
+
+JPGB_HD void compose16(const SegRun *seg, int ns, const ChunkRun *ch, int nc, unsigned long long x, uint32_t w[4], unsigned &raw) {
+    const unsigned long long xb = x * 8, xe = xb + 128;
+    for (int i = first_ending_after(nc, xb, [&](int k) { return ch[k].bit0 + ch[k].bits; }); i < nc; ++i) {
+        const ChunkRun c = ch[i];
+        if (c.bit0 >= xe) break;
+        if (c.bits == 0) continue;
+        const long long sb = (long long)(xb - c.bit0);
+        const long long a = sb >> 5;
+        const unsigned s = (unsigned)(sb & 31);
+        const long long nw = (c.bits + 31) >> 5;
+        uint32_t v[5];
+JPGB_UNROLL
+        for (int k = 0; k < 5; ++k) v[k] = (a + k >= 0 && a + k < nw) ? load_pool(c.src + (a + k)) : 0u;
+        const long long end = (long long)(c.bit0 + c.bits - xb);
+JPGB_UNROLL
+        for (int k = 0; k < 4; ++k) {
+            uint32_t g = fshl(v[k + 1], v[k], s);
+            const long long e = end - 32 * k;
+            if (e < 32) g = e <= 0 ? 0u : g & ~(0xFFFFFFFFu >> (unsigned)e);
+            w[k] |= g;
+        }
+    }
+    for (int i = first_ending_after(ns, x, [&](int k) { return seg[k].hi; }); i < ns; ++i) {
+        const SegRun r = seg[i];
+        if (r.lo >= x + 16) break;
+        const unsigned long long d1 = (r.pbit + 7) >> 3;
+        for (unsigned long long p = r.lo > x ? r.lo : x; p < x + 16 && p < r.hi; ++p) {
+            uint32_t byte;
+            if (p < r.d0) byte = r.lead ? r.lead[p - r.lo] : (r.mark >> (8 * (unsigned)(p - r.lo))) & 0xFFu;
+            else if (p >= d1) byte = p == d1 ? 0xFFu : 0xD9u;
+            else {
+                p = d1 - 1;
+                continue;
+            }
+            const unsigned j = (unsigned)(p - x);
+            or_byte(w, j, byte);
+            raw |= 1u << j;
+        }
+        const unsigned pb = (unsigned)(r.pbit & 7);
+        if (pb) {
+            const unsigned long long p = r.pbit >> 3;
+            if (p >= x && p < x + 16) {
+                or_byte(w, (unsigned)(p - x), 0xFFu >> pb);
+            }
+        }
+    }
+}
+
+JPGB_HD uint32_t ff_flags(uint32_t v) {
+    const uint32_t y = ~v;
+    const uint32_t t = ((y & 0x7F7F7F7Fu) + 0x7F7F7F7Fu) | y;
+    return ~t & 0x80808080u;
+}
+JPGB_HD unsigned flags_to_nibble(uint32_t z) { return (((z >> 7) * 0x00204081u) >> 21) & 0xFu; }
+
+JPGB_HD unsigned data_ff16(const uint32_t w[4], unsigned raw, uint32_t le[4]) {
+    unsigned m = 0;
+JPGB_UNROLL
+    for (int k = 0; k < 4; ++k) {
+        le[k] = bswap(w[k]);
+        m |= flags_to_nibble(ff_flags(le[k])) << (4 * k);
+    }
+    return m & ~raw;
+}
+
+struct SerialSearch {
+    template <class Key>
+    JPGB_HD unsigned long long operator()(unsigned long long lo, unsigned long long hi, Key key, unsigned long long x) const {
+        while (lo < hi) {
+            const unsigned long long mid = (lo + hi + 1) >> 1;
+            if (key(mid) <= x) lo = mid;
+            else hi = mid - 1;
+        }
+        return lo;
+    }
+};
+
+template <class L, class LastLE = SerialSearch>
+JPGB_HD void find_piece_start(const L &l, unsigned long long x0, unsigned long long &g, unsigned long long &c, LastLE last_le = LastLE()) {
+    g = last_le(0, l.n_segs() - 1, [&](unsigned long long i) { return l.seg_lo(i); }, x0);
+    const unsigned long long c0 = l.seg_chunk0(g), cps = l.seg_cps(g), d0 = l.seg_data0(g);
+    if (x0 < d0) {
+        c = c0;
+        return;
+    }
+    const unsigned long long base = l.chunk_pos(c0), rel = (x0 - d0) * 8;
+    c = c0 + last_le(0, cps, [&](unsigned long long j) { return l.chunk_pos(c0 + j) - base; }, rel);
+}
+
+}
+}
```

New measurement: 243,900, median of 6. -21.2%, worse.
